# Makiato1999/HRI-EMO

Measured on AMD Instinct MI355X. Metric: utterances/sec fwd+bwd, d=768 T_a=400 T_t=128 N_e=6, higher is better.
Workload: dtype bf16; 1 GPU; FusionWithEmotionDecoder fwd+bwd (train mode, dropout 0.1), d=768 T_a=400 T_t=128 N_e=6 H=8, 2 fusion + 2 decoder layers, all-False masks (BASELINE cfg2); global_batch=64, batch_per_gpu=64, parallelism=dp1, grad_allreduce=none, launch=hipGraph replay, streams=2

## Files before the change

### hri-emo_amd/_lib.py

```python
import ctypes
import os

_HERE = os.path.dirname(os.path.abspath(__file__))
LIB_PATH = os.environ.get("HRIEMO_LIB") or os.path.join(_HERE, "libhriemo.so")

_C = {"p": ctypes.c_void_p, "i": ctypes.c_int, "l": ctypes.c_long, "f": ctypes.c_float,
      "Q": ctypes.c_ulonglong, "I": ctypes.c_uint}

_SIGS = {
    "hriemo_gemm_bf16": ("iiiiiplplplipipliplp", "i"),
    "hriemo_gemm_force_config": ("i", "i"),
    "hriemo_gemm_debug_flags": ("i", "i"),
    "hriemo_gemm_colsum_rows": ("iiiii", "i"),
    "hriemo_gemm_plan": ("iiiiiilppp", "i"),
    "hriemo_gemm_bf16_group_tn": ("piip", "i"),
    "hriemo_gemm_bf16_split": ("iiiiiplplplpliiplp", "i"),
    "hriemo_gemm_bf16_colsum": ("iiiiiplplplplpp", "i"),
    "hriemo_mx8_scale_ld": ("i", "l"),
    "hriemo_quant_mx8": ("pliiiplplp", "i"),
    "hriemo_gemm_mx8": ("iiiplplplplplipiplp", "i"),
    "hriemo_gemm_mx8_q": ("iiiplplplplplpiplplp", "i"),
    "hriemo_gemm_mx8_force_config": ("i", "i"),
    "hriemo_attn_fwd": ("plplplplppiiiiifQpIipp", "i"),
    "hriemo_attn_fwd_q": ("plplplplppiiiiifQpIipplplp", "i"),
    "hriemo_attn_bwd": ("plplplplplplplplpppiiiiifQpIipppp", "i"),
    "hriemo_attn_fwd_varlen": ("plplplplpppiiiiifQpIipp", "i"),
    "hriemo_attn_fwd_q_varlen": ("plplplplpppiiiiifQpIipplpllp", "i"),
    "hriemo_attn_bwd_varlen": ("plplplplplplplplppppiiiiifQpIipppp", "i"),
    "hriemo_attn_mask_bytes": ("iiii", "l"),
    "hriemo_attn_bwd_single_pass": ("iiii", "i"),
    "hriemo_attn_bwd_single_pass_q": ("iiiii", "i"),
    "hriemo_attn_bwd_kv_colsum_rows": ("iiiii", "i"),
    "hriemo_attn_bwd_colsum_rows": ("iiii", "i"),
    "hriemo_attn_bwd_dq_colsum_rows": ("iiiii", "i"),
    "hriemo_attn_plan": ("iiiiiipppppp", "i"),
    "hriemo_split_bf16x3": ("pliipiip", "i"),
    "hriemo_attn_fwd_f32": ("plplplplppiiiiifQpIip", "i"),
    "hriemo_attn_probs_f32": ("plplpppiiiiifQpIip", "i"),
    "hriemo_add_ln_f32": ("ppppppiiffQpIlp", "i"),
    "hriemo_dropout_f32": ("ppliipfQpIlp", "i"),
    "hriemo_masked_mean_f32": ("pppiiip", "i"),
    "hriemo_gate_input_f32": ("pppiip", "i"),
    "hriemo_sigmoid_beta_f32": ("pppiip", "i"),
    "hriemo_fuse_f32": ("ppipippiiip", "i"),
    "hriemo_split3_f32": ("pliipiiplp", "i"),
    "hriemo_colsum_f32_workspace_bytes": ("ii", "l"),
    "hriemo_colsum_f32": ("pliiplpipp", "i"),
    "hriemo_add_ln_bwd_f32_workspace_bytes": ("ii", "l"),
    "hriemo_add_ln_bwd_f32": ("pppppppppiiiffQpIlpp", "i"),
    "hriemo_attn_bwd_f32": ("plplplplplppplplplpiiiiifQpIip", "i"),
    "hriemo_gate_dpre_f32": ("ppipipppiiip", "i"),
    "hriemo_gate_input_bwd_f32": ("pppppiip", "i"),
    "hriemo_gate_dy_f32": ("ppipppiiiip", "i"),
    "hriemo_rowdot_bwd_f32": ("ppppppiiip", "i"),
    "hriemo_attn_fwd_f32_varlen": ("plplplplpppiiiiifQpIip", "i"),
    "hriemo_attn_bwd_f32_varlen": ("plplplplplpppplplplpiiiiifQpIip", "i"),
    "hriemo_add_ln_f32_rows": ("ppppppiiffQpIlpp", "i"),
    "hriemo_add_ln_bwd_f32_rows": ("pppppppppiiiffQpIlppp", "i"),
    "hriemo_masked_mean_f32_packed": ("ppipiiip", "i"),
    "hriemo_fuse_f32_packed": ("pppiippiipppiiiip", "i"),
    "hriemo_gate_dpre_f32_packed": ("ppippiippiipppiiip", "i"),
    "hriemo_gate_dy_f32_packed": ("ppipippipiiiip", "i"),
    "hriemo_attn_probs": ("plplpppiiiiifQpIip", "i"),
    "hriemo_attn_probs_mfma": ("plplpppiiiiifQpIip", "i"),
    "hriemo_attn_probs_varlen": ("plplppppiiiiiiifQpIip", "i"),
    "hriemo_attn_probs_f32_varlen": ("plplppppiiiiiiifQpIip", "i"),
    "hriemo_add_ln_fwd": ("pppppppppiiffQpIlp", "i"),
    "hriemo_add_ln_fwd_mx8": ("pppppppppiiffQpIlpplp", "i"),
    "hriemo_add_ln_fwd_rows": ("pppppppppiiffQpIlpplpp", "i"),
    "hriemo_add_ln_bwd_rows": ("ppppppppppppiiifQpIlppp", "i"),
    "hriemo_add_ln_bwd_workspace_bytes": ("ii", "l"),
    "hriemo_add_ln_bwd": ("ppppppppppppiiifQpIlpp", "i"),
    "hriemo_colsum_workspace_bytes": ("ii", "l"),
    "hriemo_colsum_bf16": ("pliipipp", "i"),
    "hriemo_cast_f32_to_bf16": ("pplp", "i"),
    "hriemo_cast_bf16_to_f32": ("pplp", "i"),
    "hriemo_cast_f32_to_bf16_batch": ("pip", "i"),
    "hriemo_cast_copy_batch": ("pip", "i"),
    "hriemo_pack_rows": ("pppiiiipppp", "i"),
    "hriemo_unpack_rows": ("pppiiippp", "i"),
    "hriemo_dropout_bf16": ("pplifQpIlp", "i"),
    "hriemo_gemm_ln_supported": ("i", "i"),
    "hriemo_gemm_ln_fwd": ("iiiplplppppppppppffQpIlpp", "i"),
    "hriemo_expand_rows": ("pppilp", "i"),
    "hriemo_seed_bump": ("pp", "i"),
    "hriemo_rowdot_fwd": ("pppppiip", "i"),
    "hriemo_rowdot_bwd": ("pppppppiiip", "i"),
    "hriemo_pool_chunks": ("i", "i"),
    "hriemo_ln_pool_fwd": ("pppppppppiiiifp", "i"),
    "hriemo_gate_input": ("ppppiiiipppp" + "p", "i"),
    "hriemo_sigmoid_beta": ("pppiip", "i"),
    "hriemo_fuse_fwd": ("ppppiiip", "i"),
    "hriemo_add_ln_bwd_partial_rows": ("ii", "i"),
    "hriemo_rowops_force_variant": ("i", "i"),
    "hriemo_colsum_partial_rows": ("ii", "i"),
    "hriemo_colreduce_batch": ("pipip", "i"),
    "hriemo_debug_hog": ("iipp", "i"),
    "hriemo_sumsq_f32": ("plpip", "i"),
    "hriemo_adamw_flat": ("pppplfffffifpp", "i"),
    "hriemo_optim_finalize": ("pippppp", "i"),
    "hriemo_adamw_flat_dev": ("pppplppp", "i"),
    "hriemo_masked_mean_fwd": ("ppppiiip", "i"),
    "hriemo_rowsum_f32": ("ppilp", "i"),
    "hriemo_gate_input_pooled": ("pppiip", "i"),
    "hriemo_fusion_loss": ("ppppiiiffpppp", "i"),
    "hriemo_fusion_loss_ce": ("pppiiiffpppp", "i"),
    "hriemo_scalar_gate_dx": ("pipippppiiip", "i"),
    "hriemo_fuse_bwd_dw": ("ppppiiip", "i"),
    "hriemo_gate_dpre": ("pippp" + "iip", "i"),
    "hriemo_gate_input_bwd": ("ppppppiip", "i"),
    "hriemo_ln_pool_bwd_chunks": ("i", "i"),
    "hriemo_ln_pool_pair_supported": ("i", "i"),
    "hriemo_ln_pool_fwd_pair": ("pppppppppi" * 2 + "iiifp", "i"),
    "hriemo_ln_pool_bwd_pair": ("pip" + "ppppppppppip" * 2 + "iiip", "i"),
    "hriemo_ln_pool_bwd_workspace_bytes": ("iii", "l"),
    "hriemo_ln_pool_bwd": ("pipipppppppppp" + "iiiipp", "i"),
    "hriemo_ln_pool_fwd_packed": ("pppiippppppipiiifp", "i"),
    "hriemo_ln_pool_fwd_packed_pair": ("pppiippppppi" * 2 + "piiifp", "i"),
    "hriemo_fuse_fwd_packed": ("pppppiiiip", "i"),
    "hriemo_fuse_fwd_packed_q": ("pppppiiiipplp", "i"),
    "hriemo_fuse_bwd_dw_packed": ("pppppiiiip", "i"),
    "hriemo_ln_pool_bwd_packed": ("ppipippppiipppppp" + "iiiipp", "i"),
    "hriemo_ln_pool_bwd_packed_pair": ("ppip" + "ppppiippppppip" * 2 + "iiip", "i"),
    "hriemo_prof_enable": ("i", "i"),
    "hriemo_prof_nclass": ("", "i"),
    "hriemo_prof_collect": ("ippp", "i"),
    "hriemo_abi_version": ("", "i"),
}

_lib = None


def lib():
    global _lib
    if _lib is None:
        if not os.path.exists(LIB_PATH):
            raise RuntimeError(
                f"{LIB_PATH} not found: build it with `make -C hri-emo_amd/csrc` (or __graft_entry__.build()). "
                "There is no CPU/eager fallback for this path.")
        L = ctypes.CDLL(LIB_PATH)
        for name, (args, res) in _SIGS.items():
            fn = getattr(L, name)
            fn.argtypes = [_C[c] for c in args]
            fn.restype = _C[res]
        L.hriemo_last_error.restype = ctypes.c_char_p
        L.hriemo_last_error.argtypes = []
        L.hriemo_prof_name.restype = ctypes.c_char_p
        L.hriemo_prof_name.argtypes = [ctypes.c_int]
        _lib = L
    return _lib


def call(name, *args):
    L = lib()
    rc = getattr(L, name)(*args)
    if rc != 0:
        raise RuntimeError(f"{name} failed ({rc}): {L.hriemo_last_error().decode()}")
```

### hri-emo_amd/_ops.py

```python
import itertools
import os as _os
import threading
from collections import namedtuple

import torch

from . import _lib

BF16 = torch.bfloat16
_EPS = 1e-5
_apply_tls = threading.local()


def _stream():
    return torch.cuda.current_stream().cuda_stream


def _p(t):
    return None if t is None else t.data_ptr()


def _require_fp32_master(p):
    if p.dtype != torch.float32:
        raise TypeError(f"hri_emo_amd: parameter of dtype {p.dtype}; keep the module's parameters in fp32 "
                        "(the bf16 compute copies are made internally, as under torch.autocast)")


def _require_fp32_masters(*ps):
    for p in ps:
        if p is not None:
            _require_fp32_master(p)


def _require_gpu(t):
    if not t.is_cuda:
        raise RuntimeError(
            "hri_emo_amd runs on MI355X only: got a CPU tensor. There is no CPU fallback for this path "
            "(move the module and its inputs to 'cuda').")


_ws_cache = {}
_ws_retired = []
GRAPHS_ALIVE = 0


def workspace(nbytes, device, slot=0):
    key = (device.index, slot, torch.cuda.current_stream(device).cuda_stream)
    t = _ws_cache.get(key)
    if t is None or t.numel() * 4 < nbytes:
        if t is not None and GRAPHS_ALIVE > 0:
            _ws_retired.append(t)
        n = max(int(nbytes), 64 << 20) // 4 + 16
        t = torch.empty(n, dtype=torch.float32, device=device)
        _ws_cache[key] = t
    return t


_side_streams = {}
TWO_STREAMS = _os_env_flag = None


def side_stream(device):
    global TWO_STREAMS
    if TWO_STREAMS is None:
        import os
        TWO_STREAMS = os.environ.get("HRIEMO_TWO_STREAMS", "1") != "0"
    if not TWO_STREAMS:
        return None
    s = _side_streams.get(device.index)
    if s is None:
        s = torch.cuda.Stream(device=device)
        _side_streams[device.index] = s
    return s


class StepContext:
    __slots__ = ("capturing", "capture_origin", "seq_override", "join_scope", "half_reports")

    def __init__(self):
        self.capturing, self.capture_origin, self.seq_override, self.join_scope, self.half_reports = False, None, None, 0, {}


CTX = StepContext()


class use_context:

    def __init__(self, ctx):
        self.ctx, self.prev = ctx, None

    def __enter__(self):
        global CTX
        self.prev, CTX = CTX, self.ctx
        return self.ctx

    def __exit__(self, *exc):
        global CTX
        CTX = self.prev
        return False


def fork(child, parent):
    if CTX.capturing and CTX.capture_origin is not None and parent != CTX.capture_origin and child != CTX.capture_origin:
        raise RuntimeError("hri_emo_amd: a stream was forked from a stream that is itself a fork of the capture stream; ROCm 7.2 "
                           "crashes in hipStreamEndCapture on nested forks -- fork helper streams from the capturing stream only "
                           "(join the side stream back first), or run this step eagerly")
    child.wait_stream(parent)


_main_streams = {}


def note_main_stream(stream):
    _main_streams[stream.device.index] = stream


def branch_streams(device):
    out = [_main_streams.get(device.index, torch.cuda.current_stream(device))]
    side = _side_streams.get(device.index)
    if side is not None:
        out.append(side)
    return out


def share(t, stream):
    if t is not None:
        t.record_stream(stream)
    return t


class TextBranch:

    def __init__(self, side, main):
        self.side, self.main = side, main

    def fork(self, *handed):
        if self.side is not None:
            fork(self.side, self.main)
            for x in handed:
                share(x, self.side)

    def run(self):
        return torch.cuda.stream(self.side)

    def join(self, *back):
        if self.side is not None:
            self.main.wait_stream(self.side)
            for x in back:
                share(x, self.main)


_site_counter = itertools.count(1)


def new_site_base():
    return next(_site_counter) * 4


_seed_words = {}
STEP_ID = 0


def begin_step():
# ... 216 lines not shown
                    if (p.dim() < 2 or any(p is q for q in after_flush)) and _small_dw.touches(p.grad):
                        _small_dw.add_hook(hook, p, True)
                    elif (p.dim() < 2 or any(p is q for q in after_flush)) and DEFER_REDUCE and _in_backward():
                        _deferred.add_hook(hook, p)
                    elif p.dim() >= 2 and _small_dw.touches(p.grad):
                        _small_dw.add_hook(hook, p)
                    else:
                        hook(p)


def prefetch_batch(pairs):
    jobs, upd = [], []
    for sh, p in pairs:
        need, dst, ver = sh.stale(p)
        if not need:
            continue
        _require_gpu(p)
        _require_fp32_master(p)
        if not p.is_contiguous() or p.data_ptr() % 16:
            sh.get(p)
            continue
        if dst is None:
            dst = torch.empty(p.shape, dtype=BF16, device=p.device)
        jobs.append((p.data_ptr(), dst.data_ptr(), p.numel()))
        upd.append((sh, id(p), ver, dst))
    if jobs:
        host = torch.tensor(jobs, dtype=torch.int64)
        _lib.call("hriemo_cast_f32_to_bf16_batch", host.data_ptr(), len(jobs), _stream())
        for sh, key, ver, dst in upd:
            sh._d[key] = (ver, dst, STEP_ID)


def padded_shadow(sh, p, kp):
    key = (id(p), "pad")
    ent = sh._d.get(key)
    ver = (p._version, p.data_ptr(), WEIGHTS_EPOCH)
    if CTX.capturing or ent is None or ent[0] != ver or ent[1].device != p.device:
        _require_gpu(p)
        _require_fp32_master(p)
        s_ = ent[1] if ent is not None and ent[1].device == p.device else \
            torch.zeros((p.shape[0], kp), dtype=BF16, device=p.device)
        s_[:, :p.shape[1]].copy_(p.detach())
        ent = (ver, s_)
        sh._d[key] = ent
    return ent[1]


def to_bf16(x):
    return x if x.dtype == BF16 else x.to(BF16)


def mask_u8(mask, B, L):
    if mask is None:
        return None
    if mask.shape != (B, L):
        raise ValueError(f"key_padding_mask shape {tuple(mask.shape)} != {(B, L)}")
    m = mask.contiguous()
    return m.view(torch.uint8) if m.dtype == torch.bool else m.to(torch.uint8)


def gemm(ta, tb, M, N, K, A, lda, B, ldb, C, ldc, c_f32=False, bias=None, epi=0, aux=None, ldaux=0, accumulate=False):
    ws = workspace(64 << 20, C.device) if c_f32 else None
    _lib.call("hriemo_gemm_bf16", ta, tb, M, N, K, _p(A), lda, _p(B), ldb, _p(C), ldc, int(c_f32), _p(bias), epi,
              _p(aux), ldaux, int(accumulate), _p(ws), ws.numel() * 4 if ws is not None else 0, _stream())


def linear_fwd(x, w16, bias, relu=False, out_f32=False):
    M, K = x.shape
    N = w16.shape[0]
    y = torch.empty((M, N), dtype=torch.float32 if out_f32 else BF16, device=x.device)
    gemm(0, 0, M, N, K, x, x.stride(0), w16, w16.stride(0), y, N, c_f32=out_f32, bias=bias, epi=1 if relu else 0)
    return y


def linear_dx(dy, w16, epi=0, aux=None):
    M, N = dy.shape
    K = w16.shape[1]
    dx = torch.empty((M, K), dtype=BF16, device=dy.device)
    gemm(0, 1, M, K, N, dy, dy.stride(0), w16, w16.stride(0), dx, K, epi=epi, aux=aux,
         ldaux=aux.stride(0) if aux is not None else 0)
    return dx


FOLD_FFN_BIAS = True


def fold_ffn_bias():
    return FOLD_FFN_BIAS


def linear_dx_masked_colsum(dy, w16, aux, bias_out, accumulate):
    M, N = dy.shape
    K = w16.shape[1]
    dx = torch.empty((M, K), dtype=BF16, device=dy.device)
    rows = _lib.lib().hriemo_gemm_colsum_rows(0, 1, M, K, N)
    part = torch.empty(rows * K, dtype=torch.float32, device=dy.device)
    _lib.call("hriemo_gemm_bf16_colsum", 0, 1, M, K, N, _p(dy), dy.stride(0), _p(w16), w16.stride(0), _p(dx), K, _p(aux), aux.stride(0),
              _p(part), _stream())
    if accumulate and DEFER_REDUCE and _in_backward():
        _deferred.add(part, K, rows, K, 1, [bias_out], True)
    else:
        red = _DeferredReduce()
        red.device = dy.device
        red.add(part, K, rows, K, 1, [bias_out], accumulate, schedule=False)
        red.flush()
    return dx


def linear_dw(dy, x, out, accumulate=False):
    M, N = dy.shape
    K = x.shape[1]
    if accumulate and M <= SMALL_DW_ROWS and _small_dw.enabled():
        _small_dw.add(dy, x, out)
        return
    gemm(1, 1, N, K, M, dy, dy.stride(0), x, x.stride(0), out, out.stride(0), c_f32=True, accumulate=accumulate)


def linear_dw_split(dy, x, out, out2, split, accumulate=False):
    M, N = dy.shape
    K = x.shape[1]
    ws = workspace(64 << 20, out.device)
    _lib.call("hriemo_gemm_bf16_split", 1, 1, N, K, M, _p(dy), dy.stride(0), _p(x), x.stride(0), _p(out), out.stride(0), _p(out2),
              out2.stride(0), split, int(accumulate), _p(ws), ws.numel() * 4, _stream())


GEMM_MODE = None


def set_gemm_mode(mode):
    global GEMM_MODE
    if mode not in ("bf16", "mx_fp8"):
        raise ValueError(f"gemm mode {mode!r}: expected 'bf16' or 'mx_fp8'")
    GEMM_MODE = mode


def gemm_mode():
    global GEMM_MODE
    if GEMM_MODE is None:
        import os
        GEMM_MODE = os.environ.get("HRIEMO_GEMM", "bf16")
        if GEMM_MODE not in ("bf16", "mx_fp8"):
            raise ValueError(f"HRIEMO_GEMM={GEMM_MODE!r}: expected 'bf16' or 'mx_fp8'")
    return GEMM_MODE


PRECISION = None


def set_precision(mode):
    global PRECISION
    if mode not in ("bf16", "fp32"):
        raise ValueError(f"set_precision: {mode!r} (expected 'bf16' or 'fp32')")
    PRECISION = mode


def precision():
    global PRECISION
    if PRECISION is None:
        import os
        mode = os.environ.get("HRIEMO_PRECISION", "bf16")
        if mode not in ("bf16", "fp32"):
            raise ValueError(f"HRIEMO_PRECISION={mode!r} (expected 'bf16' or 'fp32')")
        PRECISION = mode
    return PRECISION


# ... 248 lines not shown
    if cu is not None:
        out = torch.empty((B,) + tuple(out_l), dtype=torch.float32, device=q.device)
        _lib.call("hriemo_attn_probs_varlen", _p(q), q.stride(0), _p(k), k.stride(0), _p(cu[0]), _p(cu[1]), _p(lse), _p(out), B, H,
                  Lq, Lk, out_l[0], out_l[1], hd, float(p), seed, _p(seed_word(q.device)), site, b_off, _stream())
        return out
    out = torch.empty((B, Lq, Lk), dtype=torch.float32, device=q.device)
    _lib.call("hriemo_attn_probs_mfma" if MFMA_MAPS else "hriemo_attn_probs", _p(q), q.stride(0), _p(k), k.stride(0), _p(kpm), _p(lse), _p(out), B, H, Lq, Lk,
              hd, float(p), seed, _p(seed_word(q.device)), site, b_off, _stream())
    return out


def add_ln_fwd(g, x, gamma, beta, p, seed, site, row_off, x32=None, want32=False, want_mx=False, rows=None):
    M, d = g.shape
    y = torch.empty((M, d), dtype=BF16, device=g.device)
    y32 = torch.empty((M, d), dtype=torch.float32, device=g.device) if want32 else None
    mean = torch.empty(M, dtype=torch.float32, device=g.device)
    rstd = torch.empty(M, dtype=torch.float32, device=g.device)
    if DROP_LOG is not None and p > 0 and rows is None:
        DROP_LOG.append(("rows", seed, site, M, d, float(p), row_off))
    if rows is not None:
        yq = ys = None
        ld = 0
        if want_mx:
            ld = _lib.lib().hriemo_mx8_scale_ld(M)
            yq = torch.empty((M, d), dtype=torch.uint8, device=g.device)
            ys = torch.empty((d // 32, ld), dtype=torch.uint8, device=g.device)
        _lib.call("hriemo_add_ln_fwd_rows", _p(g), _p(x), _p(x32), _p(gamma), _p(beta), _p(y), _p(y32), _p(mean), _p(rstd), M, d,
                  _EPS, float(p), seed, _p(seed_word(g.device)), site, row_off, _p(yq), _p(ys), ld, _p(rows), _stream())
        return (y, y32, mean, rstd, (yq, ys)) if want_mx else (y, y32, mean, rstd)
    if want_mx:
        ld = _lib.lib().hriemo_mx8_scale_ld(M)
        yq = torch.empty((M, d), dtype=torch.uint8, device=g.device)
        ys = torch.empty((d // 32, ld), dtype=torch.uint8, device=g.device)
        _lib.call("hriemo_add_ln_fwd_mx8", _p(g), _p(x), _p(x32), _p(gamma), _p(beta), _p(y), _p(y32), _p(mean), _p(rstd), M, d,
                  _EPS, float(p), seed, _p(seed_word(g.device)), site, row_off, _p(yq), _p(ys), ld, _stream())
        return y, y32, mean, rstd, (yq, ys)
    _lib.call("hriemo_add_ln_fwd", _p(g), _p(x), _p(x32), _p(gamma), _p(beta), _p(y), _p(y32), _p(mean), _p(rstd), M, d,
              _EPS, float(p), seed, _p(seed_word(g.device)), site, row_off, _stream())
    return y, y32, mean, rstd


def add_ln_bwd(dy, g, x, gamma, mean, rstd, p, seed, site, row_off, want_dx=True, outs=None, accumulate=False, x32=None, rows=None):
    M, d = g.shape
    dev = g.device
    dx = torch.empty((M, d), dtype=BF16, device=dev) if want_dx else None
    dg = torch.empty((M, d), dtype=BF16, device=dev) if (p > 0 or not want_dx) else None
    if outs is None:
        stats = torch.empty((3, d), dtype=torch.float32, device=dev)
        outs = (stats[0], stats[1], stats[2])
    L_ = _lib.lib()
    defer = accumulate and DEFER_REDUCE and _in_backward()
    if defer:
        nparts = L_.hriemo_add_ln_bwd_partial_rows(M, d)
        ws = torch.empty(nparts * 3 * d, dtype=torch.float32, device=dev)
        dests = (None, None, None, 0)
    else:
        ws = workspace(L_.hriemo_add_ln_bwd_workspace_bytes(M, d), dev, slot=1)
        dests = (_p(outs[0]), _p(outs[1]), _p(outs[2]), int(accumulate))
    _lib.call("hriemo_add_ln_bwd_rows", _p(dy), _p(g), _p(x), _p(x32), _p(gamma), _p(mean), _p(rstd), _p(dx), _p(dg), *dests, M, d,
              float(p), seed, _p(seed_word(dev)), site, row_off, _p(ws), _p(rows), _stream())
    if defer:
        _deferred.add(ws, 3 * d, nparts, d, 3 if outs[2] is not None else 2, [o for o in outs if o is not None], True)
    if dg is None:
        dg = dx
    return dx, dg, outs[0], outs[1], outs[2]


def ln_pool_fwd(x, x32, sx, gamma, beta, Yn, mean, rstd, part, sf, d):
    if sf.packed:
        _lib.call("hriemo_ln_pool_fwd_packed", _p(x), _p(x32), _p(sx.cu), sx.B, sx.N, _p(gamma), _p(beta), _p(Yn), _p(mean), _p(rstd),
                  _p(part), sx.L, _p(sf.cu), sf.N, sx.Breal, d, _EPS, _stream())
    else:
        _lib.call("hriemo_ln_pool_fwd", _p(x), _p(x32), _p(sx.kpm), _p(gamma), _p(beta), _p(Yn), _p(mean), _p(rstd), _p(part),
                  sx.B, sx.L, sf.L, d, _EPS, _stream())


def ln_pool_fwd_pair(a, t, sf, d):
    if sf.packed:
        side = lambda x, x32, sx, *rest: (_p(x), _p(x32), _p(sx.cu), sx.B, sx.N, *map(_p, rest), sx.L)
        _lib.call("hriemo_ln_pool_fwd_packed_pair", *side(*a), *side(*t), _p(sf.cu), sf.N, a[2].Breal, d, _EPS, _stream())
    else:
        side = lambda x, x32, sx, *rest: (_p(x), _p(x32), _p(sx.kpm), *map(_p, rest), sx.L)
        _lib.call("hriemo_ln_pool_fwd_pair", *side(*a), *side(*t), a[2].B, sf.L, d, _EPS, _stream())


def fuse_fwd(w, An, Tn, H, sf, d):
    if sf.packed and want_mx_copy(sf.N, d):
        ld = _lib.lib().hriemo_mx8_scale_ld(sf.N)
        hq = torch.empty((sf.N, d), dtype=torch.uint8, device=H.device)
        hs = torch.empty((d // 32, ld), dtype=torch.uint8, device=H.device)
        _lib.call("hriemo_fuse_fwd_packed_q", _p(w), _p(An), _p(Tn), _p(H), _p(sf.cu), sf.N, sf.Breal, sf.L, d, _p(hq), _p(hs), ld,
                  _stream())
        tag_mx(H, (hq, hs))
    elif sf.packed:
        _lib.call("hriemo_fuse_fwd_packed", _p(w), _p(An), _p(Tn), _p(H), _p(sf.cu), sf.N, sf.Breal, sf.L, d, _stream())
    else:
        _lib.call("hriemo_fuse_fwd", _p(w), _p(An), _p(Tn), _p(H), sf.B, sf.L, d, _stream())


def fuse_bwd_dw(dH, An, Tn, part, sf, d):
    if sf.packed:
        _lib.call("hriemo_fuse_bwd_dw_packed", _p(dH), _p(An), _p(Tn), _p(part), _p(sf.cu), sf.N, sf.Breal, sf.L, d, _stream())
    else:
        _lib.call("hriemo_fuse_bwd_dw", _p(dH), _p(An), _p(Tn), _p(part), sf.B, sf.L, d, _stream())


def ln_pool_bwd(dH, sf, w, is_a, dpool, x, x32, sx, gamma, mean, rstd, dx, dgamma, dbeta, accumulate, ws, d):
    if sf.packed:
        _lib.call("hriemo_ln_pool_bwd_packed", _p(dH), _p(sf.cu), sf.N, _p(w), is_a, _p(dpool), _p(x), _p(x32), _p(sx.cu), sx.B, sx.N,
                  _p(gamma), _p(mean), _p(rstd), _p(dx), _p(dgamma), _p(dbeta), accumulate, sx.Breal, sx.L, d, _p(ws), _stream())
    else:
        _lib.call("hriemo_ln_pool_bwd", _p(dH), sf.L, _p(w), is_a, _p(dpool), _p(sx.kpm), _p(x), _p(x32), _p(gamma), _p(mean),
                  _p(rstd), _p(dx), _p(dgamma), _p(dbeta), accumulate, sx.B, sx.L, d, _p(ws), _stream())


def ln_pool_bwd_pair(dH, sf, w, a, t, accumulate, d):
    if sf.packed:
        side = lambda ws, dpool, x, x32, sx, *rest: (_p(dpool), _p(x), _p(x32), _p(sx.cu), sx.B, sx.N, *map(_p, rest), sx.L, _p(ws))
        _lib.call("hriemo_ln_pool_bwd_packed_pair", _p(dH), _p(sf.cu), sf.N, _p(w), *side(*a), *side(*t), accumulate, a[4].Breal, d, _stream())
    else:
        side = lambda ws, dpool, x, x32, sx, *rest: (_p(dpool), _p(sx.kpm), _p(x), _p(x32), *map(_p, rest), sx.L, _p(ws))
        _lib.call("hriemo_ln_pool_bwd_pair", _p(dH), sf.L, _p(w), *side(*a), *side(*t), accumulate, a[4].B, d, _stream())


TWIN = _os.environ.get("HRIEMO_FP32_TWIN", "1") != "0"


DEFER_REDUCE = True
FOLD_ATTN_BIAS = True


class _DeferredReduce:

    def __init__(self):
        self.jobs, self.keep, self.scheduled, self.blocks, self.hooks = [], [], False, 0, []

    def _schedule(self):
        if not self.scheduled:
            torch.autograd.Variable._execution_engine.queue_callback(self.flush)
            self.scheduled = True

    def add_hook(self, hook, p):
        self.hooks.append((hook, p))
        self._schedule()

    def add(self, part, pstride, np_, w, nseg, outs, accumulate, schedule=True):
        gx = (w + 31) // 32
        self.jobs.append([part.data_ptr(), pstride, np_, w, nseg | (int(bool(accumulate)) << 8) | (self.blocks << 32)]
                         + [o.data_ptr() for o in outs] + [0] * (3 - len(outs)))
        self.blocks += gx * nseg
        self.keep.append(part)
        self.keep.extend(outs)
        self.device = part.device
        if schedule:
            self._schedule()

    def flush(self):
        jobs, n, nblocks = self.jobs, len(self.jobs), self.blocks
        self.jobs, self.scheduled, self.blocks = [], False, 0
        if n:
            host = torch.tensor(jobs, dtype=torch.int64)
            dev = torch.empty((n, 8), dtype=torch.int64, device=self.device)
            _lib.call("hriemo_colreduce_batch", host.data_ptr(), n, _p(dev), nblocks, _stream())
            self.keep.append(dev)
        if not CTX.capturing and self.keep:
            cur = torch.cuda.current_stream(self.device)
# ... 719 lines not shown
            if dkv is not None:
                dcat[:, d:].copy_(dkv)
        wq, wkv = ctx.params
        sq, skv = GradSink((wq,)), GradSink((wkv,))
        dwq = dwkv = None
        if dq is not None:
            dwq = sq.buf(wq)
            if not sq.fused:
                dwq[d:].zero_()
        if dkv is not None:
            dwkv = skv.buf(wkv)
            if not skv.fused:
                dwkv[:d].zero_()
        if dwq is not None and dwkv is not None and sq.fused == skv.fused:
            linear_dw_split(dcat, x2, dwq[:d], dwkv[d:], d, sq.fused)
        else:
            if dwq is not None:
                linear_dw(dcat[:, :d], x2, dwq[:d], sq.fused)
            if dwkv is not None:
                linear_dw(dcat[:, d:], x2, dwkv[d:], skv.fused)
        dep = None
        if ctx.join is not None:
            _, dep = ctx.join.arrive()
        dx = linear_dx(dcat, wcat, epi=3, aux=dep.view(M, d)) if dep is not None else linear_dx(dcat, wcat)
        _report_half(wq, sq)
        _report_half(wkv, skv)
        return dx.view(B, L, d), (sq.ret(dwq) if dwq is not None else None), None, (skv.ret(dwkv) if dwkv is not None else None), None, None, None, None


class KVProjFn(torch.autograd.Function):

    @staticmethod
    def forward(ctx, xkv, w_in, b_in, sh, join=None):
        _require_fp32_masters(w_in, b_in)
        _require_gpu(xkv)
        ctx.join = join
        B, Lk, d = xkv.shape
        xkv2 = _contig_bf16(xkv).view(B * Lk, d)
        w_in16 = sh.get(w_in)
        kv = proj_fwd(Operand(xkv2, mx_of(xkv)), sh, w_in, w_in16, b_in, rows=(d, 3 * d))
        ctx.save_for_backward(xkv2, w_in16)
        ctx.cfg = (B, Lk, d)
        ctx.params = (w_in,)
        return kv

    @staticmethod
    def backward(ctx, dkv):
        xkv2, w_in16 = ctx.saved_tensors
        B, Lk, d = ctx.cfg
        dkv = _contig_bf16(dkv)
        sink = GradSink(ctx.params)
        acc = sink.fused
        dw_in = sink.buf(ctx.params[0])
        if not acc:
            dw_in[:d].zero_()
        linear_dw(dkv, xkv2, dw_in[d:], acc)
        last, dep = ctx.join.arrive() if ctx.join is not None else (True, None)
        dxkv = linear_dx(dkv, w_in16[d:], epi=3, aux=dep.view(B * Lk, d)) if dep is not None else linear_dx(dkv, w_in16[d:])
        sink.done()
        if not last:
            ctx.join.deposit(dxkv)
            return None, sink.ret(dw_in), None, None, None
        return dxkv.view(B, Lk, d), sink.ret(dw_in), None, None, None


class FFNLN(_GradModeAware, torch.autograd.Function):

    @staticmethod
    def forward(ctx, x, x32, w1, b1, w2, b2, gamma, beta, sh, p, p_mid, seed, site, b_off, seq):
        seq.holds(x)
        if seq.packed and p_mid > 0:
            raise ValueError("FFNLN: packed rows with a mid-FFN dropout are not built (the encoder's FFNs have none)")
        if precision() == "fp32":
            return _fp32().ffn_ln(ctx, x, x32, w1, b1, w2, b2, gamma, beta, sh, p, p_mid, seed, site, b_off, seq)
        _require_fp32_masters(w1, b1, w2, b2, gamma, beta)
        ctx.set_materialize_grads(False)
        _require_gpu(x)
        B, L, d = x.shape
        M = B * L
        x2 = _contig_bf16(x).view(M, d)
        x32 = _c32(x32)
        x32v = x32.view(M, d) if x32 is not None else None
        w1_16, w2_16 = sh.get(w1), sh.get(w2)
        h = proj_fwd(Operand(x2, mx_of(x)), sh, w1, w1_16, b1, relu=True, want_q=p_mid == 0)
        hd_ = h
        if p_mid > 0:
            hd_ = torch.empty_like(h)
            if DROP_LOG is not None:
                DROP_LOG.append(("rows", seed, site + 2, M, h.shape[1], float(p_mid), b_off * L))
            _lib.call("hriemo_dropout_bf16", _p(h), _p(hd_), M, h.shape[1], float(p_mid), seed, _p(seed_word(h.device)),
                      site + 2, b_off * L, _stream())
        g, y, y32, mean, rstd, mx = _proj_ln(hd_, sh, w2, w2_16, b2, x2, x32v, gamma, beta, p, seed, site + 1, b_off * seq.L, seq.idx)
        ctx.save_for_backward(x2, x32v, h, hd_, g, mean, rstd, w1_16, w2_16, gamma)
        ctx.cfg = (B, L, d, p, p_mid, seed, site, b_off)
        ctx.seq = seq
        ctx.params = (w1, b1, w2, b2, gamma, beta)
        return tag_mx(y.view(B, L, d), mx), (y32.view(B, L, d) if y32 is not None else None)

    @staticmethod
    def backward(ctx, dy, dy32):
        if getattr(ctx, "fp32", False):
            return _fp32().ffn_ln_bwd(ctx, dy, dy32)
        x2, x32v, h, hd_, g, mean, rstd, w1_16, w2_16, gamma = ctx.saved_tensors
        B, L, d, p, p_mid, seed, site, b_off = ctx.cfg
        M, F = h.shape
        dev = x2.device
        p_w1, p_b1, p_w2 = ctx.params[:3]
        sink, ds, dg, dgamma, dbeta, db2 = _ln_bwd(ctx.params, dy, dy32, g, x2, x32v, gamma, mean, rstd, p, seed, site + 1,
                                                   b_off * ctx.seq.L, ctx.seq.idx)
        acc = sink.fused
        dw2 = sink.buf(p_w2)
        linear_dw(dg, hd_, dw2, acc)
        db1 = sink.buf(p_b1)
        fold = p_mid == 0 and fold_ffn_bias()
        if fold:
            da = linear_dx_masked_colsum(dg, w2_16, h, db1, acc)
        else:
            da = linear_dx(dg, w2_16, epi=2, aux=h)
        if p_mid > 0:
            _lib.call("hriemo_dropout_bf16", _p(da), _p(da), M, F, float(p_mid), seed, _p(seed_word(dev)), site + 2, b_off * L,
                      _stream())
        dw1 = sink.buf(p_w1)
        linear_dw(da, x2, dw1, acc)
        if not fold:
            colsum(da, db1, acc)
        dx = linear_dx(da, w1_16, epi=3, aux=ds)
        sink.done()
        r = sink.ret
        return (dx.view(B, L, d), None, r(dw1), r(db1), r(dw2), r(db2), r(dgamma), r(dbeta)) + (None,) * 7


class BetaGateFn(_GradModeAware, torch.autograd.Function):

    @staticmethod
    def forward(ctx, h_a, h_a32, h_t, h_t32, ga, ba, gt, bt, w1, b1, w2, b2, sh, sa, st, sf):
        if not (sa.packed == st.packed == sf.packed):
            raise ValueError("BetaGate: the three layouts must be all padded or all packed")
        B, La, Lt, d = sa.Breal, sa.L, st.L, h_a.shape[-1]
        Ra, Rt = h_a.shape[0] * h_a.shape[1], h_t.shape[0] * h_t.shape[1]
        if Ra != sa.N or Rt != st.N:
            raise ValueError(f"BetaGate: packed rows {Ra} / {Rt} do not match the plan ({sa.N} / {st.N})")
        L = La if La == Lt else Lt
        if La < L:
            raise RuntimeError(f"BetaGate: audio length {La} < text length {Lt}; the reference cannot fuse this either")
        if precision() == "fp32":
            return _fp32().beta_gate(ctx, h_a, h_a32, h_t, h_t32, ga, ba, gt, bt, w1, b1, w2, b2, sh, sa, st, sf)
        _require_fp32_masters(ga, ba, gt, bt, w1, b1, w2, b2)
        _require_gpu(h_a)
        h_a32, h_t32 = _c32(h_a32), _c32(h_t32)
        dev = h_a.device
        xa, xt = _contig_bf16(h_a), _contig_bf16(h_t)
        f32 = dict(dtype=torch.float32, device=dev)
        L_ = _lib.lib()
        nca, nct = L_.hriemo_pool_chunks(La), L_.hriemo_pool_chunks(Lt)
        An = torch.empty(sf.shape(d), dtype=BF16, device=dev)
        Tn = torch.empty(sf.shape(d), dtype=BF16, device=dev)
        mean_a, rstd_a = torch.empty(Ra, **f32), torch.empty(Ra, **f32)
        mean_t, rstd_t = torch.empty(Rt, **f32), torch.empty(Rt, **f32)
        pa, pt = torch.empty((B, nca, d), **f32), torch.empty((B, nct, d), **f32)
        st_ = _stream()
        side_a = (xa, h_a32, sa, ga, ba, An, mean_a, rstd_a, pa)
        side_t = (xt, h_t32, st, gt, bt, Tn, mean_t, rstd_t, pt)
        main = torch.cuda.current_stream(dev)
        side = side_stream(dev) if GATE_TWO_STREAMS else None
        if GATE_PAIR and L_.hriemo_ln_pool_pair_supported(d):
            ln_pool_fwd_pair(side_a, side_t, sf, d)
        elif side is not None and side != main:
            fork(side, main)
            with torch.cuda.stream(side):
                ln_pool_fwd(*side_t, sf, d)
            ln_pool_fwd(*side_a, sf, d)
            main.wait_stream(side)
            if not CTX.capturing:
                for t_ in (xt, h_t32, st.kpm, Tn, mean_t, rstd_t, pt):
                    share(t_, side)
        else:
            ln_pool_fwd(*side_a, sf, d)
            ln_pool_fwd(*side_t, sf, d)
        gin = torch.empty((B, 4 * d), dtype=BF16, device=dev)
        a_pool, t_pool = torch.empty((B, d), **f32), torch.empty((B, d), **f32)
        cnt = torch.empty((B, 2), **f32)
        _lib.call("hriemo_gate_input", _p(pa), _p(pt), _p(sa.kpm), _p(st.kpm), B, La, Lt, d, _p(gin), _p(a_pool),
                  _p(t_pool), _p(cnt), st_)
        w1_16, w2_16 = sh.get(w1), sh.get(w2)
        hid = linear_fwd(gin, w1_16, b1, relu=True)
        pre = linear_fwd(hid, w2_16, b2, out_f32=True)
        w = torch.empty((B, d), **f32)
        beta = torch.empty((B, 1), **f32)
        _lib.call("hriemo_sigmoid_beta", _p(pre), _p(w), _p(beta), B, d, st_)
        H = torch.empty(sf.shape(d), dtype=BF16, device=dev)
        fuse_fwd(w, An, Tn, H, sf, d)
        ctx.save_for_backward(xa, xt, An, Tn, mean_a, rstd_a, mean_t, rstd_t, gin, a_pool, t_pool, cnt, hid, w, w1_16,
                              w2_16, ga, gt, h_a32, h_t32)
        ctx.seqs = (sa, st, sf)
        ctx.params = (ga, ba, gt, bt, w1, b1, w2, b2)
        return H, beta

    @staticmethod
    def backward(ctx, dH, dbeta):
        if getattr(ctx, "fp32", False):
            return _fp32().beta_gate_bwd(ctx, dH, dbeta)
        (xa, xt, An, Tn, mean_a, rstd_a, mean_t, rstd_t, gin, a_pool, t_pool, cnt, hid, w, w1_16, w2_16, ga, gt,
         h_a32, h_t32) = ctx.saved_tensors
        sa, st, sf = ctx.seqs
        B, La, Lt, L, d = sa.Breal, sa.L, st.L, st.L, xa.shape[-1]
        dev = xa.device
        f32 = dict(dtype=torch.float32, device=dev)
        st_ = _stream()
        L_ = _lib.lib()
        p_ga, p_ba, p_gt, p_bt, p_w1, p_b1, p_w2, p_b2 = ctx.params
        sink = GradSink(ctx.params)
        acc = sink.fused
        dH2 = _contig_bf16(dH) if dH is not None else torch.zeros(An.shape, dtype=BF16, device=dev)
        dbeta2 = dbeta.contiguous().float() if dbeta is not None else None
        part = torch.empty((B, L_.hriemo_pool_chunks(L), d), **f32)
        fuse_bwd_dw(dH2, An, Tn, part, sf, d)
        dpre = torch.empty((B, d), dtype=BF16, device=dev)
        _lib.call("hriemo_gate_dpre", _p(part), L, _p(dbeta2), _p(w), _p(dpre), B, d, st_)
        dw2 = sink.buf(p_w2)
        linear_dw(dpre, hid, dw2, acc)
        db2 = sink.buf(p_b2)
        colsum(dpre, db2, acc)
        dhid = linear_dx(dpre, w2_16, epi=2, aux=hid)
        dw1 = sink.buf(p_w1)
        linear_dw(dhid, gin, dw1, acc)
        db1 = sink.buf(p_b1)
        colsum(dhid, db1, acc)
        dgin = linear_dx(dhid, w1_16)
        da, dt = torch.empty((B, d), **f32), torch.empty((B, d), **f32)
        _lib.call("hriemo_gate_input_bwd", _p(dgin), _p(a_pool), _p(t_pool), _p(cnt), _p(da), _p(dt), B, d, st_)
        dxa = torch.empty(sa.shape(d), dtype=BF16, device=dev)
        dxt = torch.empty(st.shape(d), dtype=BF16, device=dev)
        dga, dba, dgt, dbt = sink.buf(p_ga), sink.buf(p_ba), sink.buf(p_gt), sink.buf(p_bt)
        defer = acc and DEFER_REDUCE and _in_backward()
        nba, nbt = L_.hriemo_ln_pool_bwd_workspace_bytes(B, La, d), L_.hriemo_ln_pool_bwd_workspace_bytes(B, Lt, d)

        def one_side(is_a, dpool, x, x32, sx, gamma, mean, rstd, dx, dgam, dbet, nbytes):
            wsx = torch.empty(nbytes // 4 + 16, **f32) if defer else workspace(nbytes, dev, slot=1)
            outs_ = (None, None, 1) if defer else (dgam, dbet, int(acc))
            ln_pool_bwd(dH2, sf, w, is_a, dpool, x, x32, sx, gamma, mean, rstd, dx, *outs_, wsx, d)
            if defer:
                _deferred.add(wsx, 2 * d, B * L_.hriemo_ln_pool_bwd_chunks(sx.L), d, 2, [dgam, dbet], True)

        side_a = (da, xa, h_a32, sa, ga, mean_a, rstd_a, dxa)
        side_t = (dt, xt, h_t32, st, gt, mean_t, rstd_t, dxt)
        main = torch.cuda.current_stream(dev)
        side = side_stream(dev) if GATE_TWO_STREAMS else None
        if GATE_PAIR and L_.hriemo_ln_pool_pair_supported(d):
# ... 271 lines not shown
```

### hri-emo_amd/csrc/gemm.hip

```cpp
#include "gemm_common.h"
#include <string.h>
#include <stdlib.h>

template <int TA, int TB, int OUTF32, int BM, int BN, int WM, int WN, int NS, int BK>
__device__ __forceinline__ void gemm_body(const GemmArgs& p) {
  constexpr int NWAVE = WM * WN;
  constexpr bool K32 = (BK == 32), STAG = K32 && (WM * WN == 8);
  constexpr int A_BYTES = BM * BK * 2, B_BYTES = BN * BK * 2, STAGE = A_BYTES + B_BYTES;
  constexpr int A_PW = A_BYTES / 1024 / NWAVE, B_PW = B_BYTES / 1024 / NWAVE, LPT = A_PW + B_PW;
  constexpr int MT = BM / WM / 16, NTL = BN / WN / 16;
  static_assert(A_PW * NWAVE * 1024 == A_BYTES && B_PW * NWAVE * 1024 == B_BYTES, "tile must split evenly over waves");
  static_assert(NS >= 2 && NS <= 8 && (NS - 1) * LPT < 64, "ring depth / vmcnt range");
  static_assert(!STAG || NS == 4, "staggered schedule: 4 ring slots");
  static_assert(!K32 || NS >= 3, "32-deep stages need a ring of 3");
  extern __shared__ __attribute__((aligned(16))) char smem[];
  const int tid = threadIdx.x, lane = tid & 63;
  const int wave = __builtin_amdgcn_readfirstlane(tid >> 6);
  const int wm = wave / WN, wn = wave % WN;
  char* scratch = smem + NS * STAGE + wave * 2048;

  const int G = gridDim.x, nxcd = min(8, G), q = G / nxcd, r = G - q * nxcd;
  const int xcd = blockIdx.x % nxcd, lb = blockIdx.x / nxcd, nx = q + (xcd < r ? 1 : 0);
  const int before = xcd * q + min(xcd, r);
  const int tiles = p.tiles_m * p.tiles_n;
  const long total = (long)tiles * p.splitk;
  const int end = (int)(total * (before + nx) / G);
  const int beg = (int)(total * before / G);
  const bool dyn = p.sched != nullptr;
  unsigned* const qctr = p.sched + xcd;
  int* const qslot = (int*)(smem + NS * STAGE);
  auto leave = [&]() {
    if (dyn && tid == 0) {
      const unsigned done = atomicAdd(p.sched + 8, 1u);
      if (done == gridDim.x - 1) {
#pragma unroll
        for (int k = 0; k < 9; ++k) __hip_atomic_store(p.sched + k, 0u, __ATOMIC_RELAXED, __HIP_MEMORY_SCOPE_AGENT);
      }
    }
  };
  int wg, nwg;
  if (dyn) {
    if (tid == 0) {
      const int first = (int)atomicAdd(qctr, 2u);
      qslot[0] = beg + first;
      qslot[1] = beg + first + 1;
    }
    __syncthreads();
    wg = __builtin_amdgcn_readfirstlane(qslot[0]);
    nwg = __builtin_amdgcn_readfirstlane(qslot[1]);
    __syncthreads();
  } else {
    wg = beg + lb;
    nwg = wg + nx;
  }
  if (wg >= end) { leave(); return; }

  const long astep = TA == 0 ? BK : BK * p.lda, bstep = TB == 0 ? BK : BK * p.ldb;
  const LaneOff aoff = operand_lane<TA, BM, BK>(p.lda, lane), boff = operand_lane<TB, BN, BK>(p.ldb, lane);

  auto decode = [&](int w) {
    TileInfo t;
    t.slice = w / tiles;
    const int r = w - t.slice * tiles;
    const int tm = r / p.tiles_n, tn = r - tm * p.tiles_n;
    t.m0 = tm * BM; t.n0 = tn * BN;
    const int kbeg = t.slice * p.k_per_split;
    t.kext = min(p.K, kbeg + p.k_per_split) - kbeg;
    t.nk = (t.kext + BK - 1) / BK;
    t.abase = TA == 0 ? p.A + (long)t.m0 * p.lda + kbeg : p.A + (long)kbeg * p.lda + t.m0;
    t.bbase = TB == 0 ? p.B + (long)t.n0 * p.ldb + kbeg : p.B + (long)kbeg * p.ldb + t.n0;
    t.a_valid = p.M - t.m0; t.b_valid = p.N - t.n0;
    return t;
  };
  constexpr bool REBUILD = (MT * NTL > 16);
  auto stage = [&](int s, const TileInfo& t, int kstep) {
    char* sa = smem + s * STAGE;
    const int krem = t.kext - kstep * BK;
    if (REBUILD) {
      int l2 = lane;
      asm volatile("" : "+v"(l2));
      const LaneOff ao = operand_lane<TA, BM, BK>(p.lda, l2), bo = operand_lane<TB, BN, BK>(p.ldb, l2);
      stage_operand<TA, BM, A_PW, BK>(sa, t.abase + kstep * astep, ao, p.lda, t.a_valid, krem, wave, lane);
      stage_operand<TB, BN, B_PW, BK>(sa + A_BYTES, t.bbase + kstep * bstep, bo, p.ldb, t.b_valid, krem, wave, lane);
    } else {
      stage_operand<TA, BM, A_PW, BK>(sa, t.abase + kstep * astep, aoff, p.lda, t.a_valid, krem, wave, lane);
      stage_operand<TB, BN, B_PW, BK>(sa + A_BYTES, t.bbase + kstep * bstep, boff, p.ldb, t.b_valid, krem, wave, lane);
    }
  };
// ... 154 lines not shown
            __builtin_amdgcn_s_barrier();
            load_frags(smem + cur * STAGE, 0, afA, bfA);
          } else {
            __builtin_amdgcn_s_waitcnt(0xC07F);
          }
          __builtin_amdgcn_sched_barrier(0);
          __builtin_amdgcn_s_setprio(1);
          mma(afB, bfB);
          __builtin_amdgcn_s_setprio(0);
          __builtin_amdgcn_sched_barrier(0);
        };
        for (int it = 0; it < n_steady; ++it) kstep(it, Steady());
        for (int it = n_steady; it < nk; ++it) kstep(it, Tail());
      } else {
        constexpr int MH = MT / 2;
        bf16x8 a0[MH], a1[MH], b0[NTL], b1[NTL];
        auto load_a = [&](const char* sa, int ks, int half, bf16x8 (&af)[MH]) {
#pragma unroll
          for (int mi = 0; mi < MH; ++mi)
            af[mi] = TA == 0 ? lds_row_frag<BK>(sa, wm * MT * 16 + (half * MH + mi) * 16, ks, lane)
                             : lds_tr_frag<BM * 2>(sa, wm * MT * 16 + (half * MH + mi) * 16, ks, lane);
        };
        auto load_b = [&](const char* sa, int ks, bf16x8 (&bfr)[NTL]) {
          const char* sb = sa + A_BYTES;
#pragma unroll
          for (int ni = 0; ni < NTL; ++ni)
            bfr[ni] = TB == 0 ? lds_row_frag<BK>(sb, wn * NTL * 16 + ni * 16, ks, lane) : lds_tr_frag<BN * 2>(sb, wn * NTL * 16 + ni * 16, ks, lane);
        };
        auto cluster = [&](int half, const bf16x8 (&af)[MH], const bf16x8 (&bfr)[NTL]) {
          __builtin_amdgcn_s_setprio(1);
#pragma unroll
          for (int mi = 0; mi < MH; ++mi)
#pragma unroll
            for (int ni = 0; ni < NTL; ++ni)
              acc[half * MH + mi][ni] = __builtin_amdgcn_mfma_f32_16x16x32_bf16(bfr[ni], af[mi], acc[half * MH + mi][ni], 0, 0, 0);
          __builtin_amdgcn_s_setprio(0);
          __builtin_amdgcn_sched_barrier(0);
        };
        load_a(smem + cur * STAGE, 0, 0, a0);
        load_b(smem + cur * STAGE, 0, b0);
        auto kstep = [&](int it, auto steady) {
          prefetch_s(it, steady);
          const char* sa = smem + cur * STAGE;
          __builtin_amdgcn_sched_barrier(0);
          load_a(sa, 0, 1, a1);
          cluster(0, a0, b0);
          load_a(sa, 1, 0, a0);
          load_b(sa, 1, b1);
          cluster(1, a1, b0);
          load_a(sa, 1, 1, a1);
          cluster(0, a0, b1);
          cur = (cur + 1 == NS) ? 0 : cur + 1;
          nxt = (nxt + 1 == NS) ? 0 : nxt + 1;
          if (decltype(steady)::value || it + 1 < nk) {
            retire_s(it, steady);
            __builtin_amdgcn_s_waitcnt(0xC07F);
            __builtin_amdgcn_s_barrier();
            __builtin_amdgcn_sched_barrier(0);
            load_a(smem + cur * STAGE, 0, 0, a0);
            load_b(smem + cur * STAGE, 0, b0);
          }
          cluster(1, a1, b1);
        };
        for (int it = 0; it < n_steady; ++it) kstep(it, Steady());
        for (int it = n_steady; it < nk; ++it) kstep(it, Tail());
      }
    }
    if (has_next) wait_vmcnt<(NS - 2) * LPT>();
    int drawn = end;
    if (dyn && has_next && tid == 0) drawn = beg + (int)atomicAdd(qctr, 1u);
#if defined(HRIEMO_GEMM_ABL) && (HRIEMO_GEMM_ABL & 8)
    bool skip_epilogue;
    {
      float sum = 0.f;
#pragma unroll
      for (int a = 0; a < MT; ++a)
#pragma unroll
        for (int b = 0; b < NTL; ++b) sum += acc[a][b][0] + acc[a][b][1] + acc[a][b][2] + acc[a][b][3];
      skip_epilogue = sum != 12345.678f;
    }
    if (skip_epilogue) {
    } else
#endif
    if (OUTF32) {
      store_tile<1, 0, MT, NTL>(acc, p, T, scratch, wm, wn, lane);
    } else {
      switch (p.epi) {
        case 1: store_tile<0, 1, MT, NTL>(acc, p, T, scratch, wm, wn, lane); break;
        case 2: store_tile<0, 2, MT, NTL>(acc, p, T, scratch, wm, wn, lane); break;
        case 3: store_tile<0, 3, MT, NTL>(acc, p, T, scratch, wm, wn, lane); break;
        default: store_tile<0, 0, MT, NTL>(acc, p, T, scratch, wm, wn, lane); break;
      }
    }
    if (!has_next) break;
    if (!OUTF32) {
      const int rows_valid = p.M - (T.m0 + wm * MT * 16), cols_valid = p.N - (T.n0 + wn * 64);
      relax_first = (p.flags & 1) && rows_valid >= MT * 16 && cols_valid >= 64 && p.cs == nullptr;
    }
    T = decode(nwg);
    wg = nwg;
    if (dyn) {
      if (tid == 0) qslot[0] = drawn;
      __builtin_amdgcn_s_waitcnt(0xC07F);
      parked = true;
    } else {
      nwg = wg + nx;
    }
  }
  leave();
}

template <int TA, int TB, int OUTF32, int BM, int BN, int WM, int WN, int NS, int BK>
__global__ __launch_bounds__(WM * WN * 64, (WM * WN == 4 ? 2 : 1)) void gemm_kernel(const GemmArgs p) {
  gemm_body<TA, TB, OUTF32, BM, BN, WM, WN, NS, BK>(p);
}

template <int TA, int TB, int OUTF32>
__global__ __launch_bounds__(768) void gemm_ws_kernel(const GemmArgs p) {
  constexpr int BM = 256, BN = 128, BK = 64, NS = 3, WN = 2, NCW = 8, NLW = 4, MT = 4, NTL = 4;
  constexpr int A_BYTES = BM * BK * 2, B_BYTES = BN * BK * 2, STAGE = A_BYTES + B_BYTES;
  constexpr int A_PL = A_BYTES / 1024 / NLW, B_PL = B_BYTES / 1024 / NLW, LPL = A_PL + B_PL;
  extern __shared__ __attribute__((aligned(16))) char smem[];
  const int tid = threadIdx.x, lane = tid & 63;
  const int wave = __builtin_amdgcn_readfirstlane(tid >> 6);
  const int G = gridDim.x, nxcd = min(8, G), q = G / nxcd, r = G - q * nxcd;
  const int xcd = blockIdx.x % nxcd, lb = blockIdx.x / nxcd, nx = q + (xcd < r ? 1 : 0);
  const int before = xcd * q + min(xcd, r);
  const int tiles = p.tiles_m * p.tiles_n;
  const long total = (long)tiles * p.splitk;
  const int end = (int)(total * (before + nx) / G), beg = (int)(total * before / G);
  const bool dyn = p.sched != nullptr;
  unsigned* const qctr = p.sched + xcd;
  int* const qslot = (int*)(smem + NS * STAGE);
  const int wg0 = beg + lb, wg1 = wg0 + nx;
  auto leave = [&]() {
    if (dyn && tid == 0) {
      const unsigned done = atomicAdd(p.sched + 8, 1u);
      if (done == gridDim.x - 1) {
#pragma unroll
        for (int k = 0; k < 9; ++k) __hip_atomic_store(p.sched + k, 0u, __ATOMIC_RELAXED, __HIP_MEMORY_SCOPE_AGENT);
      }
    }
  };
  if (wg0 >= end) { leave(); return; }
  auto decode = [&](int w) {
    TileInfo t;
    t.slice = w / tiles;
    const int rr = w - t.slice * tiles;
    const int tm = rr / p.tiles_n, tn = rr - tm * p.tiles_n;
    t.m0 = tm * BM; t.n0 = tn * BN;
    const int kbeg = t.slice * p.k_per_split;
    t.kext = min(p.K, kbeg + p.k_per_split) - kbeg;
    t.nk = (t.kext + BK - 1) / BK;
    t.abase = TA == 0 ? p.A + (long)t.m0 * p.lda + kbeg : p.A + (long)kbeg * p.lda + t.m0;
    t.bbase = TB == 0 ? p.B + (long)t.n0 * p.ldb + kbeg : p.B + (long)kbeg * p.ldb + t.n0;
    t.a_valid = p.M - t.m0; t.b_valid = p.N - t.n0;
    return t;
  };
  if (wave >= NCW) {
    __builtin_amdgcn_s_setprio(3);
    const int lw = wave - NCW;
    const long astep = TA == 0 ? BK : BK * p.lda, bstep = TB == 0 ? BK : BK * p.ldb;
    const LaneOff aoff = operand_lane<TA, BM, BK>(p.lda, lane), boff = operand_lane<TB, BN, BK>(p.ldb, lane);
    int ik = 0, islot = 0;
    int known_next = dyn ? end : wg1;
    bool more = true, crossed = false;
    TileInfo IT = decode(wg0);
    auto issue_next = [&]() -> bool {
      if (crossed) {
        crossed = false;
        if (known_next < end) IT = decode(known_next); else more = false;
      }
      if (!more) return false;
      char* sa = smem + islot * STAGE;
      const int krem = IT.kext - ik * BK;
      stage_operand<TA, BM, A_PL, BK>(sa, IT.abase + ik * astep, aoff, p.lda, IT.a_valid, krem, lw, lane);
      stage_operand<TB, BN, B_PL, BK>(sa + A_BYTES, IT.bbase + ik * bstep, boff, p.ldb, IT.b_valid, krem, lw, lane);
      islot = (islot + 1 == NS) ? 0 : islot + 1;
      if (++ik == IT.nk) { ik = 0; crossed = true; }
      return true;
    };
    int pending = 0;
    if (issue_next()) ++pending;
    if (issue_next()) ++pending;
    for (int w = wg0; w < end;) {
      const int nk = decode(w).nk;
      for (int it = 0; it < nk; ++it) {
        if (pending >= 2) wait_vmcnt<LPL>(); else wait_vmcnt<0>();
        __builtin_amdgcn_s_barrier();
        if (dyn && it == nk - 2) {
          const int v = *(LDS_PTR(const int))qslot;
          __builtin_amdgcn_s_waitcnt(0xC07F);
          known_next = __builtin_amdgcn_readfirstlane(v);
        }
        --pending;
        if (issue_next()) ++pending;
      }
// ... 270 lines not shown
    const long fit = workspace_bytes > 0 ? workspace_bytes / ((long)M * N * 4) : 0;
    if (want > fit) want = fit;
    if (want > 1) splitk = (int)want;
  }
  const int kper = ((K + splitk - 1) / splitk + 63) / 64 * 64;
  splitk = (K + kper - 1) / kper;
  if (K - (splitk - 1) * kper <= (kCfg[cfg].ns - 2) * kCfg[cfg].bk) cfg = 0;
  return {cfg, splitk, kper};
}
extern "C" int hriemo_gemm_plan(int ta, int tb, int M, int N, int K, int c_is_f32, long workspace_bytes, int* cfg, int* splitk,
                                int* k_per_split) {
  HRIEMO_CHECK(M > 0 && N > 0 && K > 0 && cfg != nullptr && splitk != nullptr && k_per_split != nullptr, "gemm_plan: bad arguments");
  HRIEMO_CHECK(!(ta == 1 && tb == 0), "gemm: layout (ta=1,tb=0) is not used by this path and not built");
  const GemmPlan pl = plan_gemm(ta, tb, M, N, K, c_is_f32, workspace_bytes);
  *cfg = pl.cfg; *splitk = pl.splitk; *k_per_split = pl.k_per_split;
  return 0;
}
extern "C" int hriemo_gemm_colsum_rows(int ta, int tb, int M, int N, int K) {
  const int wr = wave_rows(plan_gemm(ta, tb, M, N, K, 0, 0).cfg);
  return (M + wr - 1) / wr;
}

static int gemm_impl(int ta, int tb, int M, int N, int K, const void* A, long lda, const void* B, long ldb,
                     void* C, long ldc, int c_is_f32, const float* bias, int epilogue, const void* aux,
                     long ldaux, int accumulate, float* workspace, long workspace_bytes, float* colsum_partials, hipStream_t st,
                     void* C2 = nullptr, long ldc2 = 0, int split_m = 0) {
  HRIEMO_CHECK(M > 0 && N > 0 && K > 0, "gemm: empty problem M=%d N=%d K=%d", M, N, K);
  HRIEMO_CHECK(C2 == nullptr || (c_is_f32 && split_m > 0 && split_m < M && ldc2 % 4 == 0 && ((uintptr_t)C2 % 16) == 0),
               "gemm: a split output needs fp32 results, 0 < split_m < M and a 16-byte aligned second matrix");
  HRIEMO_CHECK(!(ta == 1 && tb == 0), "gemm: layout (ta=1,tb=0) is not used by this path and not built");
  HRIEMO_CHECK(N % 8 == 0, "gemm: N=%d must be a multiple of 8", N);
  HRIEMO_CHECK(lda % 8 == 0 && ldb % 8 == 0 && ldc % (c_is_f32 ? 4 : 8) == 0, "gemm: leading dims must keep 16-byte alignment");
  HRIEMO_CHECK(((uintptr_t)A % 16) == 0 && ((uintptr_t)B % 16) == 0 && ((uintptr_t)C % 16) == 0, "gemm: unaligned operand");
  HRIEMO_CHECK(lda < (1L << 21) && ldb < (1L << 21), "gemm: leading dimension too large for 32-bit tile offsets");
  if (ta == 0) HRIEMO_CHECK(K % 8 == 0, "gemm: K=%d must be a multiple of 8 for a K-contiguous operand", K);
  if (ta == 1) HRIEMO_CHECK(M % 8 == 0, "gemm: M=%d must be a multiple of 8 for a transposed A", M);
  HRIEMO_CHECK(c_is_f32 || (epilogue >= 0 && epilogue <= 3), "gemm: bad epilogue");
  HRIEMO_CHECK(epilogue < 2 || (aux != nullptr && ldaux % 8 == 0 && ((uintptr_t)aux % 16) == 0), "gemm: epilogue 2/3 needs a 16-byte aligned aux");
  HRIEMO_CHECK(!(c_is_f32 && epilogue != 0), "gemm: fp32 output has no activation epilogue");
  HRIEMO_CHECK(c_is_f32 || !accumulate, "gemm: accumulate needs fp32 output");

  const GemmPlan pl = plan_gemm(ta, tb, M, N, K, c_is_f32, workspace != nullptr ? workspace_bytes : 0);
  const int cfg = pl.cfg, splitk = pl.splitk;
  GemmArgs a = {};
  a.M = M; a.N = N; a.K = K;
  a.A = (const bf16_t*)A; a.lda = lda; a.B = (const bf16_t*)B; a.ldb = ldb;
  a.C = C; a.ldc = ldc; a.bias = bias; a.aux = (const bf16_t*)aux; a.ldaux = ldaux; a.epi = epilogue;
  a.tiles_m = (M + kCfg[cfg].bm - 1) / kCfg[cfg].bm; a.tiles_n = (N + kCfg[cfg].bn - 1) / kCfg[cfg].bn;
  a.ws = workspace; a.accumulate = accumulate; a.sched = nullptr;
  a.flags = g_gemm_flags;
  a.cs = colsum_partials;
  HRIEMO_CHECK(colsum_partials == nullptr || (epilogue == 2 && !c_is_f32), "gemm: column sums are built for the masked epilogue (2) with bf16 output");
  a.splitk = splitk; a.k_per_split = pl.k_per_split;
  if (C2 != nullptr && splitk == 1) {
    const char* A2 = (const char*)A + (size_t)split_m * 2;
    HRIEMO_CHECK(ta == 1, "gemm: a split output without split-K is built for the weight-gradient layout only");
    int rc = gemm_impl(ta, tb, split_m, N, K, A, lda, B, ldb, C, ldc, 1, nullptr, 0, nullptr, 0, accumulate, workspace, workspace_bytes, nullptr, st);
    if (rc != 0) return rc;
    return gemm_impl(ta, tb, M - split_m, N, K, A2, lda, B, ldb, C2, ldc2, 1, nullptr, 0, nullptr, 0, accumulate, workspace, workspace_bytes, nullptr, st);
  }

  const int cls = ta ? HP_GEMM_TN : (tb ? HP_GEMM_NN : HP_GEMM_NT);
  hriemo_prof_begin(cls, st);
  if (ta == 0 && tb == 0) {
    if (c_is_f32) launch_gemm<0, 0, 1>(a, cfg, st); else launch_gemm<0, 0, 0>(a, cfg, st);
  } else if (ta == 0 && tb == 1) {
    if (c_is_f32) launch_gemm<0, 1, 1>(a, cfg, st); else launch_gemm<0, 1, 0>(a, cfg, st);
  } else {
    if (c_is_f32) launch_gemm<1, 1, 1>(a, cfg, st); else launch_gemm<1, 1, 0>(a, cfg, st);
  }
  HRIEMO_LAUNCH_CHECK("gemm_kernel");
  if (splitk > 1) {
    const long nv = (long)M * N / 4;
    int grid = (int)((nv + 255) / 256);
    if (grid > 16 * hriemo_num_cus()) grid = 16 * hriemo_num_cus();
    hipLaunchKernelGGL(splitk_reduce_kernel, dim3(grid), dim3(256), 0, st, workspace, (float*)C, ldc, M, N, splitk,
                       accumulate, (float*)C2, ldc2, C2 != nullptr ? split_m : M);
    HRIEMO_LAUNCH_CHECK("splitk_reduce_kernel");
  }
  hriemo_prof_end(cls, st, 2.0 * M * N * K);
  return 0;
}

extern "C" int hriemo_gemm_bf16(int ta, int tb, int M, int N, int K, const void* A, long lda, const void* B, long ldb,
                                void* C, long ldc, int c_is_f32, const float* bias, int epilogue, const void* aux,
                                long ldaux, int accumulate, float* workspace, long workspace_bytes, hipStream_t st) {
  return gemm_impl(ta, tb, M, N, K, A, lda, B, ldb, C, ldc, c_is_f32, bias, epilogue, aux, ldaux, accumulate, workspace, workspace_bytes,
                   nullptr, st);
}
extern "C" int hriemo_gemm_bf16_split(int ta, int tb, int M, int N, int K, const void* A, long lda, const void* B, long ldb,
                                      void* C, long ldc, void* C2, long ldc2, int split_m, int accumulate, float* workspace,
                                      long workspace_bytes, hipStream_t st) {
  HRIEMO_CHECK(C2 != nullptr, "gemm_split: second output missing");
  return gemm_impl(ta, tb, M, N, K, A, lda, B, ldb, C, ldc, 1, nullptr, 0, nullptr, 0, accumulate, workspace, workspace_bytes, nullptr, st,
                   C2, ldc2, split_m);
}
extern "C" int hriemo_gemm_bf16_group_tn(const void* jobs_host, int njobs, int accumulate, hipStream_t st) {
  HRIEMO_CHECK(jobs_host != nullptr && njobs > 0, "gemm_group: empty job table");
  const long long* h = (const long long*)jobs_host;
  constexpr int BM = 128, BN = 128;
  using KernelT = void (*)(const GemmGroup);
  KernelT kern = gemm_group_kernel<1, 1, 1, BM, BN, 2, 2, 2, 64>;
  const int lds = kCfg[0].lds + 4 * 2048;
  static bool attr_set = false;
  if (!attr_set) {
    hipFuncSetAttribute((const void*)kern, hipFuncAttributeMaxDynamicSharedMemorySize, lds);
    attr_set = true;
  }
  for (int j0 = 0; j0 < njobs; j0 += 16) {

    GemmGroup g = {};
    const int nj = njobs - j0 < 16 ? njobs - j0 : 16;
    int gx = 1;
    double flops = 0.0;
    for (int j = 0; j < nj; ++j) {
      const long long* r = h + (long)(j0 + j) * 9;
      GemmArgs& a = g.p[j];
      a.M = (int)r[0]; a.N = (int)r[1]; a.K = (int)r[2];
      a.A = (const bf16_t*)r[3]; a.lda = (long)r[4]; a.B = (const bf16_t*)r[5]; a.ldb = (long)r[6]; a.C = (void*)r[7]; a.ldc = (long)r[8];
      HRIEMO_CHECK(a.M > 0 && a.N > 0 && a.K > 0 && a.M % 8 == 0 && a.N % 8 == 0, "gemm_group: job %d: bad shape %dx%dx%d", j0 + j, a.M, a.N, a.K);
      HRIEMO_CHECK(a.lda % 8 == 0 && a.ldb % 8 == 0 && a.ldc % 4 == 0 && ((uintptr_t)a.A % 16) == 0 && ((uintptr_t)a.B % 16) == 0 &&
                       ((uintptr_t)a.C % 16) == 0 && a.lda < (1L << 21) && a.ldb < (1L << 21), "gemm_group: job %d: alignment", j0 + j);
      HRIEMO_CHECK(a.K > (kCfg[0].ns - 2) * kCfg[0].bk, "gemm_group: job %d: reduction too short for the operand ring", j0 + j);
      a.tiles_m = (a.M + BM - 1) / BM; a.tiles_n = (a.N + BN - 1) / BN;
      a.splitk = 1; a.k_per_split = (a.K + 63) / 64 * 64;
      a.accumulate = accumulate; a.sched = nullptr;
      const int tiles = a.tiles_m * a.tiles_n;
      if (tiles > gx) gx = tiles;
      flops += 2.0 * a.M * a.N * a.K;
    }
    for (int j = nj; j < 16; ++j) { g.p[j] = g.p[0]; g.p[j].tiles_m = 0; g.p[j].tiles_n = 0; }
    const int cap = 2 * hriemo_num_cus();
    if (gx > cap) gx = cap;
    hriemo_prof_begin(HP_GEMM_TN, st);
    hipLaunchKernelGGL(kern, dim3(gx, nj), dim3(256), lds, st, g);
    HRIEMO_LAUNCH_CHECK("gemm_group_kernel");
    hriemo_prof_end(HP_GEMM_TN, st, flops);
  }
  return 0;
}
extern "C" int hriemo_gemm_bf16_colsum(int ta, int tb, int M, int N, int K, const void* A, long lda, const void* B, long ldb,
                                       void* C, long ldc, const void* aux, long ldaux, float* colsum_partials, hipStream_t st) {
  HRIEMO_CHECK(colsum_partials != nullptr, "gemm_colsum: partials buffer missing");
  return gemm_impl(ta, tb, M, N, K, A, lda, B, ldb, C, ldc, 0, nullptr, 2, aux, ldaux, 0, nullptr, 0, colsum_partials, st);
}
```

### hri-emo_amd/csrc/gemm_common.h

```cpp
#pragma once
#include "common.h"
#include <mutex>
#include <type_traits>

struct GemmArgs {
  int M, N, K;
  const bf16_t* A; long lda;
  const bf16_t* B; long ldb;
  void* C; long ldc;
  const float* bias;
  const bf16_t* aux; long ldaux;
  int epi;
  int tiles_m, tiles_n, splitk, k_per_split;
  float* ws;
  int accumulate;
  unsigned* sched;
  int flags;
  float* cs;
  const uint8_t* SA; long ldsa;
  const uint8_t* SB; long ldsb;
  uint8_t* CQ; long ldcq;
  uint8_t* SC; long ldsc;
};

unsigned* hriemo_gemm_sched_slot(hipStream_t st);
int hriemo_num_cus();
int hriemo_gemm_debug_flags_get();

__device__ __forceinline__ int swz4(int row) { return (0x78 >> (((row >> 2) & 3) * 2)) & 3; }

template <int BK>
__device__ __forceinline__ bf16x8 lds_row_frag(const char* tile, int sub0, int ks, int lane) {
  const int row = sub0 + (lane & 15);
  if (BK == 64) {
    const int c = ks * 4 + (lane >> 4);
    return *(LDS_PTR(const bf16x8))(tile + row * 128 + ((c ^ (row & 7)) << 4));
  } else {
    const int c = lane >> 4;
    return *(LDS_PTR(const bf16x8))(tile + row * 64 + ((c ^ swz4(row)) << 4));
  }
}

template <int ROWB>
__device__ __forceinline__ bf16x8 lds_tr_frag(const char* tile, int sub0, int ks, int lane) {
  const int g = lane >> 4, i = lane & 15, qq = i >> 2, pp = i & 3;
  const int kr = ks * 32 + 8 * g + qq;
  const int key = qq | ((g & 1) << 2);
  const int c = ((sub0 >> 3) ^ (key << 1)) | (pp >> 1);
  const char* a0 = tile + kr * ROWB + c * 16 + (pp & 1) * 8;
  s16x4 lo = __builtin_amdgcn_ds_read_tr16_b64_v4i16((LDS_PTR(s16x4))a0);
  s16x4 hi = __builtin_amdgcn_ds_read_tr16_b64_v4i16((LDS_PTR(s16x4))(a0 + 4 * ROWB));
  typedef __attribute__((ext_vector_type(8))) short s16x8;
  s16x8 r = {lo[0], lo[1], lo[2], lo[3], hi[0], hi[1], hi[2], hi[3]};
  return __builtin_bit_cast(bf16x8, r);
}

#define OOB_OFF 0x80000000u

struct LaneOff { unsigned a, b; };

__device__ __forceinline__ void lds_dma16(unsigned lds_addr, __attribute__((ext_vector_type(4))) int rsrc, unsigned voff, int soff) {
  asm volatile("s_mov_b32 m0, %0\n\ts_nop 0\n\tbuffer_load_dwordx4 %1, %2, %3 offen lds"
               :
               : "s"(lds_addr), "v"(voff), "s"(rsrc), "s"(soff)
               : "memory", "m0");
}

template <int T, int ROWS, int BK>
__device__ __forceinline__ LaneOff operand_lane(long ld, int lane) {
  LaneOff lo;
  if (T == 0) {
    if (BK == 64) {
      const int row = lane >> 3;
      lo.a = (unsigned)((row * ld + ((lane & 7) ^ row) * 8) * 2);
    } else {
      const int row = lane >> 2;
      lo.a = (unsigned)((row * ld + ((lane & 3) ^ swz4(row)) * 8) * 2);
    }
    lo.b = 0;
  } else {
    constexpr int CPR = ROWS / 8;
    const int lr = lane / CPR, lc = lane % CPR;
    lo.a = (unsigned)(lr * ld * 2);
    lo.b = (unsigned)((lc ^ (lr << 1)) << 4);
  }
  return lo;
}

template <int T, int ROWS, int PW, int BK>
__device__ __forceinline__ void stage_operand(char* tile, const bf16_t* kbase, const LaneOff lo, long ld, int valid, int krem, int wave, int lane) {
  typedef __attribute__((ext_vector_type(4))) int i32x4;
  const unsigned long kb = (unsigned long)kbase;
  const i32x4 rsrc = {(int)(unsigned)kb, (int)((kb >> 32) & 0xffffu), (int)OOB_OFF, 0x00020000};
  const bool full = valid >= ROWS && krem >= BK;
  constexpr int CPR = ROWS / 8;
  constexpr int RPI = 64 / CPR;
  constexpr int RPJ = BK == 64 ? 8 : 16;
  if (full) {
#pragma unroll
    for (int t = 0; t < PW; ++t) {
      const int j = wave * PW + t;
      if (T == 0) {
        lds_dma16((unsigned)(unsigned long)(LDS_PTR(char))(tile + j * 1024), rsrc, lo.a, (int)(j * RPJ * 2 * ld));
      } else {
        const int kr0 = j * RPI;
        const int ukey = (kr0 & 3) | (((kr0 >> 3) & 1) << 2);
        lds_dma16((unsigned)(unsigned long)(LDS_PTR(char))(tile + j * 1024), rsrc, lo.a + (lo.b ^ (unsigned)(ukey << 5)), (int)(kr0 * 2 * ld));
      }
    }
    return;
  }
#pragma unroll
  for (int t = 0; t < PW; ++t) {
    const int j = wave * PW + t;
    unsigned o;
    int so;
    if (T == 0) {
      o = lo.a;
      so = (int)(j * RPJ * 2 * ld);
      const int row = j * RPJ + (BK == 64 ? (lane >> 3) : (lane >> 2));
      const int c = BK == 64 ? ((lane & 7) ^ (row & 7)) : ((lane & 3) ^ swz4(row));
      if (row >= valid || c * 8 >= krem) o = OOB_OFF;
    } else {
      const int kr0 = j * RPI;
      const int ukey = (kr0 & 3) | (((kr0 >> 3) & 1) << 2);
      const unsigned cb = lo.b ^ (unsigned)(ukey << 5);
      o = lo.a + cb;
      so = (int)(kr0 * 2 * ld);
      if ((int)(cb >> 1) >= valid || kr0 + lane / CPR >= krem) o = OOB_OFF;
    }
    lds_dma16((unsigned)(unsigned long)(LDS_PTR(char))(tile + j * 1024), rsrc, o, so);
  }
}

template <int N> __device__ __forceinline__ void wait_vmcnt() { asm volatile("s_waitcnt vmcnt(%0)" ::"n"(N) : "memory"); }

struct TileInfo {
  const bf16_t* abase;
  const bf16_t* bbase;
  int m0, n0, slice, a_valid, b_valid, kext, nk;
};

typedef __attribute__((ext_vector_type(2))) unsigned u32x2;
typedef __attribute__((ext_vector_type(4))) unsigned u32x4;
typedef __attribute__((ext_vector_type(4))) short s16x4v;
typedef __attribute__((ext_vector_type(8))) short s16x8v;

template <int OUTF32, int EPI, int MT, int NTL>
__device__ __forceinline__ void store_tile(f32x4 (&acc)[MT][NTL], const GemmArgs& p, const TileInfo& T, char* scratch,
                                           int wm, int wn, int lane_in) {
  static_assert(NTL == 4, "wave tiles are 64 columns wide");
  int lane = lane_in;
  asm volatile("" : "+v"(lane));
  const int g = lane >> 4, i = lane & 15;
  if (OUTF32) {
#pragma unroll
    for (int mi = 0; mi < MT; ++mi) {
      const int m = T.m0 + wm * MT * 16 + mi * 16 + i;
      if (m >= p.M) continue;
#pragma unroll
      for (int ni = 0; ni < NTL; ++ni) {
        const int n = T.n0 + wn * NTL * 16 + ni * 16 + 4 * g;
        if (n >= p.N) continue;
        f32x4 v = acc[mi][ni];
        if (p.bias != nullptr && T.slice == 0) v += *(const f32x4*)(p.bias + n);
        float* dst = p.splitk > 1 ? p.ws + ((long)T.slice * p.M + m) * p.N + n : (float*)p.C + (long)m * p.ldc + n;
        if (p.splitk == 1 && p.accumulate) v += *(const f32x4*)dst;
        *(f32x4*)dst = v;
      }
    }
  } else {
    const int mb = T.m0 + wm * MT * 16, nb = T.n0 + wn * 64;
    const int rows_valid = p.M - mb, cols_valid = p.N - nb;
    const bool full = rows_valid >= MT * 16 && cols_valid >= 64;
    const int rr = lane >> 3, cc = lane & 7;
    char* cbase = (char*)((bf16_t*)p.C + (long)mb * p.ldc + nb);
    const unsigned line_c = (unsigned)((rr * p.ldc + cc * 8) * 2);

    f32x4 b4[NTL];
#pragma unroll
    for (int ni = 0; ni < NTL; ++ni) {
      const int n = nb + ni * 16 + 4 * g;
      b4[ni] = (p.bias != nullptr && n < p.N) ? *(const f32x4*)(p.bias + n) : (f32x4){0.f, 0.f, 0.f, 0.f};
    }
    constexpr int CM = MT >= 8 ? 2 : MT;
    constexpr int NCH = MT / CM;
    __amdgpu_buffer_rsrc_t rx = __builtin_amdgcn_make_buffer_rsrc((void*)(EPI >= 2 ? p.aux + (long)mb * p.ldaux + nb : (const bf16_t*)p.C), 0, (int)OOB_OFF, 0x00020000);
    const unsigned frag_x = (unsigned)((i * p.ldaux + 4 * g) * 2);
    const unsigned line_x = (cc * 8 < cols_valid) ? (unsigned)((rr * p.ldaux + cc * 8) * 2) : OOB_OFF;
    u32x2 ax[2][EPI == 3 ? CM : 1][NTL];
    u32x4 al[2][EPI == 2 ? CM : 1][2];
    auto load_chunk = [&](int c, int buf) {
#pragma unroll
      for (int q = 0; q < CM; ++q) {
        const int mi = c * CM + q;
        if (EPI == 3) {
#pragma unroll
          for (int ni = 0; ni < NTL; ++ni) {
            const bool ok = full || (mi * 16 + i < rows_valid && ni * 16 + 4 * g < cols_valid);
            ax[buf][q][ni] = __builtin_amdgcn_raw_buffer_load_b64(rx, ok ? (int)frag_x : (int)OOB_OFF, (int)((mi * 16 * p.ldaux + ni * 16) * 2), 0);
          }
        }
        if (EPI == 2) {
#pragma unroll
          for (int k = 0; k < 2; ++k) {
            const bool ok = full || mi * 16 + k * 8 + rr < rows_valid;
            al[buf][q][k] = __builtin_amdgcn_raw_buffer_load_b128(rx, ok ? (int)line_x : (int)OOB_OFF, (int)((mi * 16 + k * 8) * p.ldaux * 2), 0);
          }
        }
      }
    };
    char* wr = scratch + i * 128 + (g & 1) * 8;
    const int wsw = i & 7, gh = g >> 1;
    const char* rd0 = scratch + rr * 128 + ((cc ^ rr) << 4);
    if (EPI >= 2) load_chunk(0, 0);
    float cs8[EPI == 2 ? 8 : 1];
#pragma unroll
    for (int e = 0; e < (EPI == 2 ? 8 : 1); ++e) cs8[e] = 0.f;
#pragma unroll
    for (int c = 0; c < NCH; ++c) {
      if (EPI >= 2 && c + 1 < NCH) load_chunk(c + 1, (c + 1) & 1);
#pragma unroll
      for (int q = 0; q < CM; ++q) {
        const int mi = c * CM + q;
#pragma unroll
        for (int ni = 0; ni < NTL; ++ni) {
          f32x4 v = acc[mi][ni] + b4[ni];
          if (EPI == 3) {
            const bf16x4 a4 = __builtin_bit_cast(bf16x4, ax[c & 1][q][ni]);
#pragma unroll
            for (int e = 0; e < 4; ++e) v[e] += (float)a4[e];
          }
          bf16x4 o = __builtin_convertvector(v, bf16x4);
          if (EPI == 1) {
            const s16x4v z = {0, 0, 0, 0};
            o = __builtin_bit_cast(bf16x4, __builtin_elementwise_max(__builtin_bit_cast(s16x4v, o), z));
          }
          *(LDS_PTR(bf16x4))(wr + (((ni * 2 + gh) ^ wsw) << 4)) = o;
        }
        asm volatile("s_waitcnt lgkmcnt(0)" ::: "memory");
        u32x4 ln[2];
#pragma unroll
        for (int k = 0; k < 2; ++k) ln[k] = *(LDS_PTR(const u32x4))(rd0 + k * 1024);
#pragma unroll
        for (int k = 0; k < 2; ++k) {
          u32x4 v = ln[k];
          if (EPI == 2) {
            const s16x8v z = {0, 0, 0, 0, 0, 0, 0, 0};
            const s16x8v neg = __builtin_elementwise_sub_sat(z, __builtin_bit_cast(s16x8v, al[c & 1][q][k]));
            v &= __builtin_bit_cast(u32x4, neg >> 15);
            asm volatile("" : "+v"(v));
            if (p.cs != nullptr) {
              const bf16x8 m8 = __builtin_bit_cast(bf16x8, v);
#pragma unroll
              for (int e = 0; e < 8; ++e) cs8[e] += (float)m8[e];
            }
          }
          const bool ok = mi * 16 + k * 8 + rr < rows_valid && cc * 8 < cols_valid;
          if (full || ok) *(u32x4*)(cbase + (long)((mi * 16 + k * 8) * p.ldc * 2) + line_c) = v;
          if (EPI <= 1 && p.CQ != nullptr) {
            float f8[8];
            bf8_to_f32(__builtin_bit_cast(bf16x8, v), f8);
            int e;
            const __attribute__((ext_vector_type(2))) int w8 = mx8_block(f8, e);
            const long qrow = mb + mi * 16 + k * 8 + rr;
            const int qcol = nb + cc * 8;
            if (full || ok) {
              *(__attribute__((ext_vector_type(2))) int*)(p.CQ + qrow * p.ldcq + qcol) = w8;
              if ((cc & 3) == 0) p.SC[(long)(qcol >> 5) * p.ldsc + qrow] = (uint8_t)e;
            }
          }
        }
      }
    }
    if (EPI == 2 && p.cs != nullptr) {
#pragma unroll
      for (int e = 0; e < 8; ++e) {
        float t = cs8[e];
        t += __shfl_xor(t, 8);
        t += __shfl_xor(t, 16);
        t += __shfl_xor(t, 32);
        cs8[e] = t;
      }
      if (rr == 0 && mb < p.M && cc * 8 < cols_valid) {
        float* row = p.cs + (long)(mb / (MT * 16)) * p.N + nb + cc * 8;
        *(f32x4*)row = (f32x4){cs8[0], cs8[1], cs8[2], cs8[3]};
        *(f32x4*)(row + 4) = (f32x4){cs8[4], cs8[5], cs8[6], cs8[7]};
      }
    }
  }
}
```

### hri-emo_amd/csrc/rowops.hip

```cpp
#include "common.h"
#include <string.h>
#include <stdlib.h>

#define EPS_DEFAULT 1e-5f

struct RowDrop { uint64_t seed; const unsigned long long* seed_dev; uint32_t site, thr16; float inv_keep; const long long* rowmap; };
static RowDrop row_drop(float p, uint64_t seed, const unsigned long long* seed_dev, uint32_t site) {
  DropCfg d = make_drop(p, seed, site);
  RowDrop r; r.seed = seed; r.seed_dev = seed_dev; r.site = site; r.thr16 = d.thr16; r.inv_keep = d.inv_keep; r.rowmap = nullptr;
  return r;
}
__device__ __forceinline__ uint32_t row_key(const RowDrop& dr) {
  return dr.thr16 != 0 ? site_key(eff_seed(dr.seed, dr.seed_dev), dr.site, 0u) : 0u;
}

template <int NCH>
__device__ __forceinline__ void block_colsum(float* lds_row, const float (&acc)[NCH][8], int nchunk, int lane, int wave, int nwave) {
  for (int w = 0; w < nwave; ++w) {
    if (wave == w) {
#pragma unroll
      for (int c = 0; c < NCH; ++c) {
        const int ch = lane + 64 * c;
        if (ch < nchunk) {
#pragma unroll
          for (int j = 0; j < 8; ++j) {
            if (w == 0) lds_row[ch * 8 + j] = acc[c][j];
            else lds_row[ch * 8 + j] += acc[c][j];
          }
        }
      }
    }
    __syncthreads();
  }
}

__device__ __forceinline__ void row_keep8(uint32_t key32, uint32_t thr16, uint32_t row, int ch, bool (&kp)[8]) {
  if (thr16 == 0) {
#pragma unroll
    for (int j = 0; j < 8; ++j) kp[j] = true;
    return;
  }
  const uint32_t hb = drop_base(key32, row, (uint32_t)(ch * 4));
#pragma unroll
  for (int pr = 0; pr < 4; ++pr) {
    const uint32_t x = mix24(hb + (uint32_t)pr * DROP_CB);
    kp[2 * pr] = keep_lo(x, thr16);
    kp[2 * pr + 1] = keep_hi(x, thr16);
  }
}

__device__ __forceinline__ void load_resid(const bf16_t* X, const float* X32, long off, float* xf) {
  if (X32 != nullptr) {
    const f32x4 a = *(const f32x4*)(X32 + off), b = *(const f32x4*)(X32 + off + 4);
    xf[0] = a[0]; xf[1] = a[1]; xf[2] = a[2]; xf[3] = a[3]; xf[4] = b[0]; xf[5] = b[1]; xf[6] = b[2]; xf[7] = b[3];
  } else if (X != nullptr) {
    bf8_to_f32(*(const bf16x8*)(X + off), xf);
  } else {
#pragma unroll
    for (int j = 0; j < 8; ++j) xf[j] = 0.f;
  }
}

template <int NCH>
__device__ __forceinline__ void load_cols(const float* __restrict__ v, int nchunk, int lane, float (&out)[NCH][8]) {
#pragma unroll
  for (int c = 0; c < NCH; ++c) {
    const int ch = lane + 64 * c;
#pragma unroll
    for (int j = 0; j < 8; ++j) out[c][j] = 0.f;
    if (ch < nchunk) {
      const f32x4 a = *(const f32x4*)(v + ch * 8), b = *(const f32x4*)(v + ch * 8 + 4);
#pragma unroll
      for (int e = 0; e < 4; ++e) { out[c][e] = a[e]; out[c][4 + e] = b[e]; }
    }
  }
}

template <int NCH>
__global__ __launch_bounds__(256) void add_ln_fwd_kernel(const bf16_t* __restrict__ G, const bf16_t* __restrict__ X,
                                                         const float* __restrict__ X32, const float* __restrict__ gamma,
                                                         const float* __restrict__ beta, bf16_t* __restrict__ Y,
                                                         float* __restrict__ Y32, float* __restrict__ mean_o,
                                                         float* __restrict__ rstd_o, int M, int d, float eps, RowDrop dr,
                                                         long row_offset, uint8_t* __restrict__ Yq, uint8_t* __restrict__ SY, long ldsy) {
  const uint32_t key32 = row_key(dr);
// ... 571 lines not shown
    for (int c = 0; c < NCH; ++c) {
      const int ch = lane + 64 * c;
      if (ch < nchunk) load_resid(X, X32, (xbase + l) * d + ch * 8, dst[c]);
    }
  };
  if (PF && chunk * 32 + wave < lend) load_row(chunk * 32 + wave, nx);
  for (int l = chunk * 32 + wave; l < lend; l += 4) {
    const long row = xbase + l;
    float s[NCH][8];
    float sum = 0.f;
    if (!PF) load_row(l, nx);
#pragma unroll
    for (int c = 0; c < NCH; ++c) {
      const int ch = lane + 64 * c;
      if (ch < nchunk) {
#pragma unroll
        for (int j = 0; j < 8; ++j) { s[c][j] = nx[c][j]; sum += s[c][j]; }
      }
    }
    if (PF && l + 4 < lend) load_row(l + 4, nx);
    const float mu = wave_sum(sum) * invd;
    float sq = 0.f;
#pragma unroll
    for (int c = 0; c < NCH; ++c)
      if (lane + 64 * c < nchunk) {
#pragma unroll
        for (int j = 0; j < 8; ++j) { const float t = s[c][j] - mu; sq += t * t; }
      }
    const float rstd = rsqrtf(wave_sum(sq) * invd + eps);
    const bool valid = PK || mask == nullptr || mask[row] == 0;
#pragma unroll
    for (int c = 0; c < NCH; ++c) {
      const int ch = lane + 64 * c;
      if (ch < nchunk) {
        float o[8];
#pragma unroll
        for (int j = 0; j < 8; ++j) {
          o[j] = (s[c][j] - mu) * rstd * (HOIST ? gm8[HOIST ? c : 0][j] : gamma[ch * 8 + j]) + (HOIST ? bt8[HOIST ? c : 0][j] : beta[ch * 8 + j]);
          if (valid) acc[c][j] += o[j];
        }
        if (l < Lkeep) *(bf16x8*)(Yn + (ybase + l) * d + ch * 8) = f32_to_bf8(o);
      }
    }
    if (lane == 0) { mean_o[row] = mu; rstd_o[row] = rstd; }
  }
  block_colsum<NCH>(red, acc, nchunk, lane, wave, 4);
  float* out = partials + ((long)b * nchunks + chunk) * d;
  for (int t = threadIdx.x; t < d; t += 256) out[t] = red[t];
}
template <int NCH, bool PF>
__global__ __launch_bounds__(256) void ln_pool_fwd_kernel(const bf16_t* __restrict__ X, const float* __restrict__ X32, const uint8_t* __restrict__ mask,
                                                          const float* __restrict__ gamma, const float* __restrict__ beta,
                                                          bf16_t* __restrict__ Yn, float* __restrict__ mean_o, float* __restrict__ rstd_o,
                                                          float* __restrict__ partials, int L, int Lkeep, int d, float eps) {
  ln_pool_fwd_body<NCH, PF>(X, X32, mask, gamma, beta, Yn, mean_o, rstd_o, partials, L, Lkeep, d, eps, blockIdx.x, gridDim.x);
}
struct PoolFwdSide { const bf16_t* X; const float* X32; const uint8_t* mask; const float* gamma; const float* beta; bf16_t* Yn; float* mean; float* rstd; float* partials; int L, Lkeep, nc; };
struct PoolFwdPair { PoolFwdSide s[2]; };
#define PAIR_PICK(f) (second ? p.s[1].f : p.s[0].f)
template <int NCH, bool PF>
__global__ __launch_bounds__(256, 4) void ln_pool_fwd_pair_kernel(const PoolFwdPair p, int d, float eps) {
  const bool second = (int)blockIdx.x >= p.s[0].nc;
  ln_pool_fwd_body<NCH, PF>(PAIR_PICK(X), PAIR_PICK(X32), PAIR_PICK(mask), PAIR_PICK(gamma), PAIR_PICK(beta), PAIR_PICK(Yn), PAIR_PICK(mean),
                            PAIR_PICK(rstd), PAIR_PICK(partials), PAIR_PICK(L), PAIR_PICK(Lkeep), d, eps,
                            (int)blockIdx.x - (second ? p.s[0].nc : 0), PAIR_PICK(nc));
}
template <int NCH, bool PF>
__global__ __launch_bounds__(256) void ln_pool_fwd_packed_kernel(const bf16_t* __restrict__ X, const float* __restrict__ X32,
                                                                 const float* __restrict__ gamma, const float* __restrict__ beta,
                                                                 bf16_t* __restrict__ Yn, float* __restrict__ mean_o, float* __restrict__ rstd_o,
                                                                 float* __restrict__ partials, int L, int d, float eps, const PackedArgs pk) {
  ln_pool_fwd_body<NCH, PF, true>(X, X32, nullptr, gamma, beta, Yn, mean_o, rstd_o, partials, L, 0, d, eps, blockIdx.x, gridDim.x, pk);
}
struct PoolFwdSidePk { const bf16_t* X; const float* X32; const int* cu; const float* gamma; const float* beta; bf16_t* Yn; float* mean; float* rstd; float* partials; int L, nc, nseq, n_rows; };
struct PoolFwdPairPk { PoolFwdSidePk s[2]; };
template <int NCH, bool PF>
__global__ __launch_bounds__(256, 4) void ln_pool_fwd_packed_pair_kernel(const PoolFwdPairPk p, const int* __restrict__ cu_f, int n_f, int B, int d, float eps) {
  const bool second = (int)blockIdx.x >= p.s[0].nc;
  if ((int)blockIdx.y > PAIR_PICK(nseq)) return;
  const PackedArgs pk{PAIR_PICK(cu), PAIR_PICK(nseq), PAIR_PICK(n_rows), cu_f, n_f, B};
  ln_pool_fwd_body<NCH, PF, true>(PAIR_PICK(X), PAIR_PICK(X32), nullptr, PAIR_PICK(gamma), PAIR_PICK(beta), PAIR_PICK(Yn), PAIR_PICK(mean),
                                  PAIR_PICK(rstd), PAIR_PICK(partials), PAIR_PICK(L), 0, d, eps,
                                  (int)blockIdx.x - (second ? p.s[0].nc : 0), PAIR_PICK(nc), pk);
}

__global__ __launch_bounds__(256) void gate_input_kernel(const float* __restrict__ pa, int nca, const float* __restrict__ pt, int nct,
                                                         const uint8_t* __restrict__ mask_a, const uint8_t* __restrict__ mask_t, int La, int Lt,
                                                         int d, bf16_t* __restrict__ gin, float* __restrict__ a_pool, float* __restrict__ t_pool,
                                                         float* __restrict__ cnt) {
  __shared__ float sc[2], wc[4][2];
  const int b = blockIdx.x, tid = threadIdx.x;
  float ca = 0.f, ct = 0.f;
  for (int l = tid; l < La; l += 256) ca += (mask_a == nullptr || mask_a[(long)b * La + l] == 0) ? 1.f : 0.f;
  for (int l = tid; l < Lt; l += 256) ct += (mask_t == nullptr || mask_t[(long)b * Lt + l] == 0) ? 1.f : 0.f;
  ca = wave_sum(ca); ct = wave_sum(ct);
  if ((tid & 63) == 0) { wc[tid >> 6][0] = ca; wc[tid >> 6][1] = ct; }
  __syncthreads();
  if (tid == 0) {
    sc[0] = fmaxf(wc[0][0] + wc[1][0] + wc[2][0] + wc[3][0], 1.f); sc[1] = fmaxf(wc[0][1] + wc[1][1] + wc[2][1] + wc[3][1], 1.f);
    cnt[b * 2] = sc[0]; cnt[b * 2 + 1] = sc[1];
  }
  __syncthreads();
  const float ia = 1.f / sc[0], it = 1.f / sc[1];
  for (int c = tid; c < d; c += 256) {
    float a = 0.f, t = 0.f;
    for (int k0 = 0; k0 < nca; k0 += 8) {
      float v[8];
#pragma unroll
      for (int k = 0; k < 8; ++k) v[k] = k0 + k < nca ? pa[((long)b * nca + k0 + k) * d + c] : 0.f;
#pragma unroll
      for (int k = 0; k < 8; ++k) if (k0 + k < nca) a += v[k];
    }
    for (int k0 = 0; k0 < nct; k0 += 8) {
      float v[8];
#pragma unroll
      for (int k = 0; k < 8; ++k) v[k] = k0 + k < nct ? pt[((long)b * nct + k0 + k) * d + c] : 0.f;
#pragma unroll
      for (int k = 0; k < 8; ++k) if (k0 + k < nct) t += v[k];
    }
    a *= ia; t *= it;
    a_pool[(long)b * d + c] = a; t_pool[(long)b * d + c] = t;
    bf16_t* g = gin + (long)b * 4 * d;
    g[c] = (bf16_t)a; g[d + c] = (bf16_t)t; g[2 * d + c] = (bf16_t)fabsf(a - t); g[3 * d + c] = (bf16_t)(a * t);
  }
}

__global__ __launch_bounds__(256) void sigmoid_beta_kernel(const float* __restrict__ pre, float* __restrict__ w, float* __restrict__ beta, int d) {
  __shared__ float red[4];
  const int b = blockIdx.x, tid = threadIdx.x;
  float s = 0.f;
  for (int c = tid; c < d; c += 256) {
    const float v = 1.f / (1.f + __expf(-pre[(long)b * d + c]));
    w[(long)b * d + c] = v;
    s += v;
  }
  s = wave_sum(s);
  if ((tid & 63) == 0) red[tid >> 6] = s;
  __syncthreads();
  if (tid == 0) beta[b] = (red[0] + red[1] + red[2] + red[3]) / (float)d;
}

__global__ void fuse_fwd_kernel(const float* __restrict__ w, const bf16_t* __restrict__ A, const bf16_t* __restrict__ T,
                                bf16_t* __restrict__ H, int B, int L, int d) {
  const int nch = d >> 3;
  const long nv = (long)B * L * nch;
  for (long v = (long)blockIdx.x * blockDim.x + threadIdx.x; v < nv; v += (long)gridDim.x * blockDim.x) {
    const int ch = (int)(v % nch);
    const long b = v / ((long)L * nch);
    float a[8], t[8], o[8];
    bf8_to_f32(*(const bf16x8*)(A + v * 8), a);
    bf8_to_f32(*(const bf16x8*)(T + v * 8), t);
    const float* wp = w + b * d + ch * 8;
#pragma unroll
    for (int j = 0; j < 8; ++j) o[j] = wp[j] * a[j] + (1.f - wp[j]) * t[j];
    *(bf16x8*)(H + v * 8) = f32_to_bf8(o);
  }
}

template <int NCH, bool MXQ = false>
__global__ __launch_bounds__(256) void fuse_fwd_packed_kernel(const float* __restrict__ w, const bf16_t* __restrict__ A, const bf16_t* __restrict__ T,
                                                              bf16_t* __restrict__ H, const int* __restrict__ cu_f, int n_f, int B, int L, int d,
                                                              uint8_t* __restrict__ Hq = nullptr, uint8_t* __restrict__ Hs = nullptr, long lds = 0) {
  typedef __attribute__((ext_vector_type(2))) int i32x2;
  const int lane = threadIdx.x & 63, wave = threadIdx.x >> 6;
  const int b = blockIdx.y, chunk = blockIdx.x, nchunk = d >> 3;
  if (b == B) {
// ... 753 lines not shown
                                                                bf16_t* __restrict__ gin, int d) {
  const int b = blockIdx.x;
  bf16_t* g = gin + (long)b * 4 * d;
  for (int c = threadIdx.x; c < d; c += 256) {
    const float a = a_pool[(long)b * d + c], t = t_pool[(long)b * d + c];
    g[c] = (bf16_t)a; g[d + c] = (bf16_t)t; g[2 * d + c] = (bf16_t)fabsf(a - t); g[3 * d + c] = (bf16_t)(a * t);
  }
}

__global__ __launch_bounds__(256) void sumsq_f32_kernel(const float* __restrict__ x, long n, float* __restrict__ partial) {
  __shared__ float red[4];
  float s = 0.f;
  const long nv = n >> 2;
  for (long v = (long)blockIdx.x * 256 + threadIdx.x; v < nv; v += (long)gridDim.x * 256) {
    const f32x4 t = *(const f32x4*)(x + v * 4);
    s += t[0] * t[0] + t[1] * t[1] + t[2] * t[2] + t[3] * t[3];
  }
  s = wave_sum(s);
  if ((threadIdx.x & 63) == 0) red[threadIdx.x >> 6] = s;
  __syncthreads();
  if (threadIdx.x == 0) partial[blockIdx.x] = red[0] + red[1] + red[2] + red[3];
}

__global__ __launch_bounds__(256) void adamw_flat_kernel(float* __restrict__ p, const float* __restrict__ g, float* __restrict__ m,
                                                         float* __restrict__ v, long n, float lr, float b1, float b2, float eps,
                                                         float wd, float bc1, float bc2, float max_norm, const float* __restrict__ norm2) {
  float coef = 1.f;
  if (max_norm > 0.f) coef = fminf(1.f, max_norm / (sqrtf(norm2[0]) + 1e-6f));
  const float step = lr / bc1, isb2 = 1.f / sqrtf(bc2);
  const long nv = n >> 2;
  for (long i = (long)blockIdx.x * 256 + threadIdx.x; i < nv; i += (long)gridDim.x * 256) {
    f32x4 pp = *(const f32x4*)(p + i * 4), mm = *(const f32x4*)(m + i * 4), vv = *(const f32x4*)(v + i * 4);
    const f32x4 gg = *(const f32x4*)(g + i * 4) * coef;
#pragma unroll
    for (int e = 0; e < 4; ++e) {
      pp[e] *= 1.f - lr * wd;
      mm[e] += (gg[e] - mm[e]) * (1.f - b1);
      vv[e] = vv[e] * b2 + gg[e] * gg[e] * (1.f - b2);
      pp[e] -= step * mm[e] / (sqrtf(vv[e]) * isb2 + eps);
    }
    *(f32x4*)(p + i * 4) = pp; *(f32x4*)(m + i * 4) = mm; *(f32x4*)(v + i * 4) = vv;
  }
}

extern "C" int hriemo_pool_chunks(int L) { return (L + 31) / 32; }

extern "C" int hriemo_ln_pool_fwd(const void* X, const float* X32, const unsigned char* mask, const float* gamma, const float* beta, void* Yn,
                                  float* mean, float* rstd, float* partials, int B, int L, int Lkeep, int d, float eps,
                                  hipStream_t st) {
  if (check_rows(B * L, d)) return 1;
  HRIEMO_CHECK(Lkeep >= 0 && Lkeep <= L, "ln_pool_fwd: Lkeep=%d out of range (L=%d)", Lkeep, L);
  const int nc = (L + 31) / 32;
  hriemo_prof_begin(HP_ROWOPS, st);
#define CALL(N)                                                                                                                  \
  if ((N) <= 2)                                                                                                                  \
    hipLaunchKernelGGL((ln_pool_fwd_kernel<N, ((N) <= 2)>), dim3(nc, B), dim3(256), d * 4, st, (const bf16_t*)X, X32, mask, gamma, beta, (bf16_t*)Yn, mean, rstd, partials, L, Lkeep, d, eps); \
  else                                                                                                                           \
    hipLaunchKernelGGL((ln_pool_fwd_kernel<N, false>), dim3(nc, B), dim3(256), d * 4, st, (const bf16_t*)X, X32, mask, gamma, beta, (bf16_t*)Yn, mean, rstd, partials, L, Lkeep, d, eps)
  DISPATCH_NCH(d, CALL)
#undef CALL
  HRIEMO_LAUNCH_CHECK("ln_pool_fwd_kernel");
  hriemo_prof_end(HP_ROWOPS, st, ((double)B * L + (double)B * Lkeep) * d * 2);
  return 0;
}

extern "C" int hriemo_ln_pool_pair_supported(int d) { return d % 8 == 0 && d <= 1024 ? 1 : 0; }
extern "C" int hriemo_ln_pool_fwd_pair(const void* Xa, const float* Xa32, const unsigned char* mask_a, const float* gamma_a, const float* beta_a,
                                       void* Yna, float* mean_a, float* rstd_a, float* partials_a, int La,
                                       const void* Xt, const float* Xt32, const unsigned char* mask_t, const float* gamma_t, const float* beta_t,
                                       void* Ynt, float* mean_t, float* rstd_t, float* partials_t, int Lt,
                                       int B, int Lkeep, int d, float eps, hipStream_t st) {
  if (check_rows(B * La, d) || check_rows(B * Lt, d)) return 1;
  HRIEMO_CHECK(Lkeep >= 0 && Lkeep <= La && Lkeep <= Lt, "ln_pool_fwd_pair: Lkeep=%d out of range (La=%d, Lt=%d)", Lkeep, La, Lt);
  HRIEMO_CHECK(hriemo_ln_pool_pair_supported(d), "ln_pool_fwd_pair: d=%d (pairs are built for d <= 1024; use two hriemo_ln_pool_fwd calls)", d);
  PoolFwdPair p;
  p.s[0] = PoolFwdSide{(const bf16_t*)Xa, Xa32, mask_a, gamma_a, beta_a, (bf16_t*)Yna, mean_a, rstd_a, partials_a, La, Lkeep, (La + 31) / 32};
  p.s[1] = PoolFwdSide{(const bf16_t*)Xt, Xt32, mask_t, gamma_t, beta_t, (bf16_t*)Ynt, mean_t, rstd_t, partials_t, Lt, Lkeep, (Lt + 31) / 32};
  const int nc = p.s[0].nc + p.s[1].nc;
  hriemo_prof_begin(HP_ROWOPS, st);
  if (d <= 512) hipLaunchKernelGGL((ln_pool_fwd_pair_kernel<1, true>), dim3(nc, B), dim3(256), d * 4, st, p, d, eps);
  else hipLaunchKernelGGL((ln_pool_fwd_pair_kernel<2, true>), dim3(nc, B), dim3(256), d * 4, st, p, d, eps);
  HRIEMO_LAUNCH_CHECK("ln_pool_fwd_pair_kernel");
  hriemo_prof_end(HP_ROWOPS, st, ((double)B * (La + Lt) + 2.0 * B * Lkeep) * d * 2);
  return 0;
}

extern "C" int hriemo_gate_input(const float* partials_a, const float* partials_t, const unsigned char* mask_a,
                                 const unsigned char* mask_t, int B, int La, int Lt, int d, void* gate_in, float* a_pool,
                                 float* t_pool, float* cnt, hipStream_t st) {
  HRIEMO_CHECK(B > 0 && d > 0, "gate_input: empty");
  hipLaunchKernelGGL(gate_input_kernel, dim3(B), dim3(256), 0, st, partials_a, (La + 31) / 32, partials_t, (Lt + 31) / 32, mask_a,
                     mask_t, La, Lt, d, (bf16_t*)gate_in, a_pool, t_pool, cnt);
  HRIEMO_LAUNCH_CHECK("gate_input_kernel");
  return 0;
}

extern "C" int hriemo_sigmoid_beta(const float* pre, float* w, float* beta, int B, int d, hipStream_t st) {
  HRIEMO_CHECK(B > 0 && d > 0, "sigmoid_beta: empty");
  hipLaunchKernelGGL(sigmoid_beta_kernel, dim3(B), dim3(256), 0, st, pre, w, beta, d);
  HRIEMO_LAUNCH_CHECK("sigmoid_beta_kernel");
  return 0;
}

extern "C" int hriemo_masked_mean_fwd(const void* X, const unsigned char* mask, float* pooled, float* cnt, int B, int L, int d,
                                      hipStream_t st) {
  if (check_rows(B * L, d)) return 1;
  hriemo_prof_begin(HP_ROWOPS, st);
  hipLaunchKernelGGL(masked_mean_fwd_kernel, dim3((d / 8 + 63) / 64, B), dim3(256), 0, st, (const bf16_t*)X, mask, pooled, cnt, L, d);
  HRIEMO_LAUNCH_CHECK("masked_mean_fwd_kernel");
  hriemo_prof_end(HP_ROWOPS, st, 1.0 * B * L * d * 2);
  return 0;
}

extern "C" int hriemo_gate_input_pooled(const float* a_pool, const float* t_pool, void* gate_in, int B, int d, hipStream_t st) {
  HRIEMO_CHECK(B > 0 && d > 0, "gate_input_pooled: empty");
  hipLaunchKernelGGL(gate_input_pooled_kernel, dim3(B), dim3(256), 0, st, a_pool, t_pool, (bf16_t*)gate_in, d);
  HRIEMO_LAUNCH_CHECK("gate_input_pooled_kernel");
  return 0;
}

extern "C" int hriemo_rowsum_f32(const float* x, float* out, int B, long n, hipStream_t st) {
  HRIEMO_CHECK(B > 0 && n > 0, "rowsum_f32: empty problem");
  hipLaunchKernelGGL(rowsum_f32_kernel, dim3(B), dim3(256), 0, st, x, out, n);
  HRIEMO_LAUNCH_CHECK("rowsum_f32_kernel");
  return 0;
}

extern "C" int hriemo_scalar_gate_dx(const void* dH, int Lf, const float* beta, int is_a, const float* dpool, const float* cnt,
                                     const unsigned char* mask, void* dX, int B, int L, int d, hipStream_t st) {
  if (check_rows(B * L, d)) return 1;
  HRIEMO_CHECK(Lf >= 0 && Lf <= L, "scalar_gate_dx: Lf=%d out of range (L=%d)", Lf, L);
  long g = ((long)B * L * (d / 8) + 255) / 256;
  if (g > 8192) g = 8192;
  hriemo_prof_begin(HP_ROWOPS, st);
  hipLaunchKernelGGL(scalar_gate_dx_kernel, dim3((int)g), dim3(256), 0, st, (const bf16_t*)dH, Lf, beta, is_a, dpool, cnt, mask,
                     (bf16_t*)dX, B, L, d);
  HRIEMO_LAUNCH_CHECK("scalar_gate_dx_kernel");
  hriemo_prof_end(HP_ROWOPS, st, 2.0 * B * L * d * 2);
  return 0;
}

extern "C" int hriemo_sumsq_f32(const float* x, long n, float* partial, int nblocks, hipStream_t st) {
  HRIEMO_CHECK(n > 0 && n % 4 == 0 && nblocks > 0 && nblocks <= 4096, "sumsq_f32: n=%ld must be a positive multiple of 4, 0 < nblocks <= 4096", n);
  HRIEMO_CHECK(((uintptr_t)x % 16) == 0, "sumsq_f32: unaligned buffer");
  hipLaunchKernelGGL(sumsq_f32_kernel, dim3(nblocks), dim3(256), 0, st, x, n, partial);
  HRIEMO_LAUNCH_CHECK("sumsq_f32_kernel");
  return 0;
}

extern "C" int hriemo_adamw_flat(float* p, const float* g, float* m, float* v, long n, float lr, float beta1, float beta2, float eps,
                                 float weight_decay, int step, float max_norm, const float* norm2, hipStream_t st) {
  HRIEMO_CHECK(n > 0 && n % 4 == 0 && step >= 1, "adamw_flat: n=%ld must be a positive multiple of 4 and step >= 1", n);
  HRIEMO_CHECK(((uintptr_t)p % 16) == 0 && ((uintptr_t)g % 16) == 0 && ((uintptr_t)m % 16) == 0 && ((uintptr_t)v % 16) == 0, "adamw_flat: unaligned buffer");
  HRIEMO_CHECK(max_norm <= 0.f || norm2 != nullptr, "adamw_flat: clipping needs the squared gradient norm");
  const float bc1 = 1.f - powf(beta1, (float)step), bc2 = 1.f - powf(beta2, (float)step);
  long gsz = (n / 4 + 255) / 256;
  if (gsz > 4096) gsz = 4096;
  hipLaunchKernelGGL(adamw_flat_kernel, dim3((int)gsz), dim3(256), 0, st, p, g, m, v, n, lr, beta1, beta2, eps, weight_decay, bc1, bc2,
                     max_norm, norm2);
  HRIEMO_LAUNCH_CHECK("adamw_flat_kernel");
  return 0;
}

extern "C" int hriemo_fuse_fwd(const float* w, const void* A, const void* T, void* H, int B, int L, int d, hipStream_t st) {
  if (check_rows(B * L, d)) return 1;
  long g = ((long)B * L * (d / 8) + 255) / 256;
// ... 233 lines not shown
```

### hri-emo_amd/models/fusion_with_emotion_decoder.py

```python
import torch
import torch.nn as nn

try:
    from .. import _ops
except ImportError:
    from hri_emo_amd import _ops
from .cross_modal_block_tacfn import CrossModalTransformer
from .beta_gate_tacfn import BetaGate
from .emotion_decoder import EmotionDecoder


class FusionWithEmotionDecoder(nn.Module):
    def __init__(self, d_model: int = 768, num_emotions: int = 4, n_heads: int = 8, num_layers_fusion: int = 2,
                 num_layers_decoder: int = 2, beta_hidden: int = 256, dropout: float = 0.1):
        super().__init__()
        self.cross_modal = CrossModalTransformer(num_layers=num_layers_fusion, d_model=d_model, n_heads=n_heads,
                                                 dropout=dropout)
        self.beta_gate = BetaGate(d_model=d_model, hidden_dim=beta_hidden)
        self.emotion_decoder = EmotionDecoder(d_model=d_model, num_emotions=num_emotions, n_heads=n_heads,
                                              num_layers=num_layers_decoder, dropout=dropout, use_output_layer=True)

    def set_batch_offset(self, offset: int):
        for m in self.modules():
            if hasattr(m, "batch_offset"):
                m.batch_offset = int(offset)

    def _prefetch_shadows(self, device):
        if _ops.precision() != "bf16" or not device.type == "cuda":
            return None
        side = _ops.side_stream(device)
        if side is None:
            return None
        main = torch.cuda.current_stream(device)
        _ops.fork(side, main)
        with torch.cuda.stream(side):
            g = self.beta_gate
            pairs = [(g._sh, g.mlp[0].weight), (g._sh, g.mlp[2].weight)]
            for layer in self.emotion_decoder.layers:
                pairs += [(layer._sh, w) for w in (layer.self_attn.in_proj_weight, layer.self_attn.out_proj.weight,
                                                   layer.cross_attn.in_proj_weight, layer.cross_attn.out_proj.weight,
                                                   layer.linear1.weight, layer.linear2.weight)]
            _ops.prefetch_batch(pairs)
            ev = torch.cuda.Event()
            ev.record(side)
        return ev

    def _ensure_3d(self, x):
        if x.dim() == 2:
            return x.unsqueeze(1)
        if x.dim() == 3:
            return x
        raise ValueError(f"Expected 2D or 3D tensor, got {x.shape}")

    def _build_fused_mask(self, mask_a, mask_t, L_fused):
        if mask_a is None and mask_t is None:
            return None

        def fit(m):
            if m is None:
                return None
            if m.size(1) < L_fused:
                pad = torch.ones(m.size(0), L_fused - m.size(1), dtype=torch.bool, device=m.device)
                return torch.cat([m, pad], dim=1)
            return m[:, :L_fused]

        ma, mt = fit(mask_a), fit(mask_t)
        if ma is None:
            return mt
        if mt is None:
            return ma
        return ma | mt

    def forward(self, h_a, h_t, mask_a=None, mask_t=None, return_attention=False):
        h_a, h_t = self._ensure_3d(h_a), self._ensure_3d(h_t)
        out_dtype = h_a.dtype
        need = bool(return_attention)
        a, a32 = _ops.as_pair(h_a)
        t, t32 = _ops.as_pair(h_t)
        _ops.begin_step()
        may_pack = _ops.varlen() and (not need or _ops.varlen_maps()) and mask_a is not None and mask_t is not None and _ops.packed_tail()
        fused_early = None if may_pack else self._build_fused_mask(mask_a, mask_t, h_t.size(1))
        ready = self._prefetch_shadows(a.device)
        _ops.CTX.join_scope += 1
        try:
            a, a32, t, t32, encoder_attns, seqs = self.cross_modal._fwd_pair(a, a32, t, t32, mask_a, mask_t, need, tail=True)
        finally:
            _ops.CTX.join_scope -= 1
        if ready is not None:
            torch.cuda.current_stream(a.device).wait_event(ready)
        h_fusion, beta = self.beta_gate._fwd_pair(a, a32, t, t32, mask_a, mask_t, seqs)
        sm = seqs[2]
        if not sm.packed:
            sm = sm.with_kpm(fused_early if (fused_early is not None and h_fusion.size(1) == h_t.size(1)) else
                             self._build_fused_mask(mask_a, mask_t, h_fusion.size(1)))
        z, logits, decoder_attns = self.emotion_decoder._fwd(h_fusion, sm, need, out_dtype)
        if return_attention:
            return logits, beta, z, {"encoder": encoder_attns, "decoder": decoder_attns}
        return logits, beta, z
```

### include/hriemo.h

```cpp
#ifndef HRIEMO_H_
#define HRIEMO_H_

#ifdef __cplusplus
extern "C" {
#endif

typedef struct ihipStream_t* hriemo_stream_t;

const char* hriemo_last_error(void);
int hriemo_abi_version(void);

int hriemo_gemm_bf16(int ta, int tb, int M, int N, int K, const void* A, long lda, const void* B, long ldb,
                     void* C, long ldc, int c_is_f32, const float* bias, int epilogue, const void* aux,
                     long ldaux, int accumulate, float* workspace, long workspace_bytes, hriemo_stream_t stream);

int hriemo_gemm_bf16_group_tn(const void* jobs_host, int njobs, int accumulate, hriemo_stream_t stream);
int hriemo_gemm_bf16_split(int ta, int tb, int M, int N, int K, const void* A, long lda, const void* B, long ldb, void* C, long ldc,
                           void* C2, long ldc2, int split_m, int accumulate, float* workspace, long workspace_bytes,
                           hriemo_stream_t stream);
int hriemo_gemm_colsum_rows(int ta, int tb, int M, int N, int K);
int hriemo_gemm_bf16_colsum(int ta, int tb, int M, int N, int K, const void* A, long lda, const void* B, long ldb, void* C, long ldc,
                            const void* aux, long ldaux, float* colsum_partials, hriemo_stream_t stream);
int hriemo_gemm_force_config(int cfg);
int hriemo_gemm_debug_flags(int flags);
int hriemo_gemm_plan(int ta, int tb, int M, int N, int K, int c_is_f32, long workspace_bytes, int* cfg, int* splitk,
                     int* k_per_split);

long hriemo_mx8_scale_ld(int rows);
int hriemo_quant_mx8(const void* X, long ldx, int src_is_f32, int M, int K, void* Xq, long ldq, void* S, long lds,
                     hriemo_stream_t stream);
int hriemo_gemm_mx8(int M, int N, int K, const void* Aq, long lda, const void* SA, long ldsa, const void* Bq, long ldb,
                    const void* SB, long ldsb, void* C, long ldc, int c_is_f32, const float* bias, int epilogue,
                    const void* aux, long ldaux, hriemo_stream_t stream);
int hriemo_gemm_mx8_q(int M, int N, int K, const void* Aq, long lda, const void* SA, long ldsa, const void* Bq, long ldb,
                      const void* SB, long ldsb, void* C, long ldc, const float* bias, int epilogue, void* CQ, long ldcq,
                      void* SC, long ldsc, hriemo_stream_t stream);
int hriemo_gemm_mx8_force_config(int cfg);

int hriemo_attn_fwd(const void* Q, long ldq, const void* K, long ldk, const void* V, long ldv, void* O, long ldo,
                    const unsigned char* key_padding_mask, float* lse, int B, int H, int Lq, int Lk, int head_dim,
                    float p_drop, unsigned long long seed, const unsigned long long* seed_dev, unsigned site, int b_offset,
                    void* drop_mask_bits, hriemo_stream_t stream);
int hriemo_attn_bwd(const void* Q, long ldq, const void* K, long ldk, const void* V, long ldv, const void* O, long ldo,
                    const void* dO, long lddo, void* dQ, long lddq, void* dK, long lddk, void* dV, long lddv,
                    const unsigned char* key_padding_mask, const float* lse, float* delta, int B, int H, int Lq,
                    int Lk, int head_dim, float p_drop, unsigned long long seed, const unsigned long long* seed_dev,
                    unsigned site, int b_offset, float* dq_colsum_partials, float* dkv_colsum_partials,
                    const void* drop_mask_bits, hriemo_stream_t stream);
long hriemo_attn_mask_bytes(int B, int H, int Lq, int Lk);
int hriemo_attn_bwd_single_pass(int B, int H, int Lk, int head_dim);
int hriemo_attn_bwd_single_pass_q(int B, int H, int Lq, int Lk, int head_dim);
int hriemo_attn_bwd_kv_colsum_rows(int B, int H, int Lq, int Lk, int head_dim);
int hriemo_attn_plan(int B, int H, int Lq, int Lk, int head_dim, int cus, int* fwd_rows, int* bwd_form, int* dq_rows, int* dkv_rows,
                     int* dq_colsum_rows, int* kv_colsum_rows);
int hriemo_attn_fwd_q(const void* Q, long ldq, const void* K, long ldk, const void* V, long ldv, void* O, long ldo,
                      const unsigned char* key_padding_mask, float* lse, int B, int H, int Lq, int Lk, int head_dim, float p_drop,
                      unsigned long long seed, const unsigned long long* seed_dev, unsigned site, int b_offset, void* drop_mask_bits,
                      void* Oq, long ldoq, void* So, long ldso, hriemo_stream_t stream);
int hriemo_attn_fwd_varlen(const void* Q, long ldq, const void* K, long ldk, const void* V, long ldv, void* O, long ldo,
                           const int* cu_seqlens_q, const int* cu_seqlens_k, float* lse, int B, int H, int max_len_q,
                           int max_len_k, int head_dim, float p_drop, unsigned long long seed, const unsigned long long* seed_dev,
                           unsigned site, int b_offset, void* drop_mask_bits, hriemo_stream_t stream);
int hriemo_attn_fwd_q_varlen(const void* Q, long ldq, const void* K, long ldk, const void* V, long ldv, void* O, long ldo,
                             const int* cu_seqlens_q, const int* cu_seqlens_k, float* lse, int B, int H, int max_len_q,
                             int max_len_k, int head_dim, float p_drop, unsigned long long seed, const unsigned long long* seed_dev,
                             unsigned site, int b_offset, void* drop_mask_bits, void* Oq, long ldoq, void* So, long ldso,
                             long n_rows, hriemo_stream_t stream);
int hriemo_attn_bwd_varlen(const void* Q, long ldq, const void* K, long ldk, const void* V, long ldv, const void* O, long ldo,
                           const void* dO, long lddo, void* dQ, long lddq, void* dK, long lddk, void* dV, long lddv,
                           const int* cu_seqlens_q, const int* cu_seqlens_k, const float* lse, float* delta, int B, int H,
                           int max_len_q, int max_len_k, int head_dim, float p_drop, unsigned long long seed,
                           const unsigned long long* seed_dev, unsigned site, int b_offset, float* dq_colsum_partials,
                           float* dkv_colsum_partials, const void* drop_mask_bits, hriemo_stream_t stream);
int hriemo_attn_bwd_colsum_rows(int B, int H, int L, int head_dim);
int hriemo_attn_bwd_dq_colsum_rows(int B, int H, int Lq, int Lk, int head_dim);
int hriemo_attn_probs(const void* Q, long ldq, const void* K, long ldk, const unsigned char* key_padding_mask,
                      const float* lse, float* probs, int B, int H, int Lq, int Lk, int head_dim, float p_drop,
                      unsigned long long seed, const unsigned long long* seed_dev, unsigned site, int b_offset,
                      hriemo_stream_t stream);
int hriemo_attn_probs_varlen(const void* Q, long ldq, const void* K, long ldk, const int* cu_seqlens_q, const int* cu_seqlens_k,
                             const float* lse, float* probs, int B, int H, int max_len_q, int max_len_k, int out_lq, int out_lk,
                             int head_dim, float p_drop, unsigned long long seed, const unsigned long long* seed_dev, unsigned site,
                             int b_offset, hriemo_stream_t stream);
int hriemo_attn_probs_mfma(const void* Q, long ldq, const void* K, long ldk, const unsigned char* key_padding_mask,
                           const float* lse, float* probs, int B, int H, int Lq, int Lk, int head_dim, float p_drop,
                           unsigned long long seed, const unsigned long long* seed_dev, unsigned site, int b_offset,
                           hriemo_stream_t stream);

int hriemo_add_ln_fwd(const void* G, const void* X, const float* X32, const float* gamma, const float* beta, void* Y,
                      float* Y32, float* mean, float* rstd, int M, int d, float eps, float p_drop, unsigned long long seed,
                      const unsigned long long* seed_dev, unsigned site, long row_offset, hriemo_stream_t stream);
int hriemo_add_ln_fwd_mx8(const void* G, const void* X, const float* X32, const float* gamma, const float* beta, void* Y,
                          float* Y32, float* mean, float* rstd, int M, int d, float eps, float p_drop, unsigned long long seed,
                          const unsigned long long* seed_dev, unsigned site, long row_offset, void* Yq, void* SY, long ldsy,
                          hriemo_stream_t stream);
int hriemo_add_ln_fwd_rows(const void* G, const void* X, const float* X32, const float* gamma, const float* beta, void* Y,
                           float* Y32, float* mean, float* rstd, int M, int d, float eps, float p_drop, unsigned long long seed,
                           const unsigned long long* seed_dev, unsigned site, long row_offset, void* Yq, void* SY, long ldsy,
                           const long long* row_index, hriemo_stream_t stream);
// ... 2 lines not shown
                           int M, int d, float p_drop, unsigned long long seed, const unsigned long long* seed_dev,
                           unsigned site, long row_offset, float* workspace, const long long* row_index, hriemo_stream_t stream);
int hriemo_pack_rows(const void* X16, const float* X32, const int* cu_seqlens, int B, int L, int d, int n_rows, void* P16, float* P32,
                     long long* row_index, hriemo_stream_t stream);
int hriemo_unpack_rows(const void* P16, const float* P32, const int* cu_seqlens, int B, int L, int d, void* Y16, float* Y32,
                       hriemo_stream_t stream);
long hriemo_add_ln_bwd_workspace_bytes(int M, int d);
int hriemo_add_ln_bwd(const void* dY, const void* G, const void* X, const float* X32, const float* gamma, const float* mean,
                      const float* rstd, void* dX, void* dG, float* dgamma, float* dbeta, float* dbias, int accumulate,
                      int M, int d, float p_drop, unsigned long long seed, const unsigned long long* seed_dev,
                      unsigned site, long row_offset, float* workspace, hriemo_stream_t stream);

long hriemo_colsum_workspace_bytes(int M, int N);
int hriemo_colsum_bf16(const void* X, long ldx, int M, int N, float* out, int accumulate, float* workspace,
                       hriemo_stream_t stream);
int hriemo_cast_f32_to_bf16(const float* src, void* dst, long n, hriemo_stream_t stream);
int hriemo_cast_bf16_to_f32(const void* src, float* dst, long n, hriemo_stream_t stream);
int hriemo_cast_f32_to_bf16_batch(const void* jobs_host, int njobs, hriemo_stream_t stream);
int hriemo_cast_copy_batch(const void* jobs_host, int njobs, hriemo_stream_t stream);
int hriemo_dropout_bf16(const void* X, void* Y, long M, int N, float p_drop, unsigned long long seed,
                        const unsigned long long* seed_dev, unsigned site, long row_offset, hriemo_stream_t stream);
int hriemo_expand_rows(const float* q, void* out, float* out32, int B, long n, hriemo_stream_t stream);
int hriemo_seed_bump(unsigned long long* seed_dev, hriemo_stream_t stream);
int hriemo_rowdot_fwd(const void* Z, const float* Z32, const float* w, const float* b, float* out, int M, int d,
                      hriemo_stream_t stream);
int hriemo_rowdot_bwd(const float* dl, const void* Z, const float* Z32, const float* w, void* dZ, float* dw, float* db, int accumulate,
                      int M, int d, hriemo_stream_t stream);

int hriemo_pool_chunks(int L);
int hriemo_ln_pool_fwd(const void* X, const float* X32, const unsigned char* mask, const float* gamma, const float* beta, void* Yn,
                       float* mean, float* rstd, float* partials, int B, int L, int Lkeep, int d, float eps,
                       hriemo_stream_t stream);
int hriemo_gate_input(const float* partials_a, const float* partials_t, const unsigned char* mask_a,
                      const unsigned char* mask_t, int B, int La, int Lt, int d, void* gate_in, float* a_pool,
                      float* t_pool, float* cnt, hriemo_stream_t stream);
int hriemo_sigmoid_beta(const float* pre, float* w, float* beta, int B, int d, hriemo_stream_t stream);
int hriemo_fuse_fwd(const float* w, const void* A, const void* T, void* H, int B, int L, int d, hriemo_stream_t stream);
int hriemo_fuse_bwd_dw(const void* dH, const void* A, const void* T, float* partials, int B, int L, int d,
                       hriemo_stream_t stream);
int hriemo_gate_dpre(const float* partials, int L, const float* dbeta, const float* w, void* dpre, int B, int d,
                     hriemo_stream_t stream);
int hriemo_gate_input_bwd(const void* dgin, const float* a_pool, const float* t_pool, const float* cnt, float* da,
                          float* dt, int B, int d, hriemo_stream_t stream);
int hriemo_masked_mean_fwd(const void* X, const unsigned char* mask, float* pooled, float* cnt, int B, int L, int d,
                           hriemo_stream_t stream);
int hriemo_rowsum_f32(const float* x, float* out, int B, long n, hriemo_stream_t stream);
int hriemo_gate_input_pooled(const float* a_pool, const float* t_pool, void* gate_in, int B, int d, hriemo_stream_t stream);
int hriemo_fusion_loss(const float* logits, const float* targets, const float* pos_weight, const float* beta, int B, int Ne,
                       int reg_mode, float reg_coef, float scale, float* loss, float* dlogits, float* dbeta, hriemo_stream_t stream);
int hriemo_fusion_loss_ce(const float* logits, const long long* labels, const float* beta, int B, int C, int reg_mode,
                          float reg_coef, float scale, float* loss, float* dlogits, float* dbeta, hriemo_stream_t stream);
int hriemo_scalar_gate_dx(const void* dH, int Lf, const float* beta, int is_a, const float* dpool, const float* cnt,
                          const unsigned char* mask, void* dX, int B, int L, int d, hriemo_stream_t stream);
int hriemo_sumsq_f32(const float* x, long n, float* partial, int nblocks, hriemo_stream_t stream);
int hriemo_adamw_flat(float* p, const float* g, float* m, float* v, long n, float lr, float beta1, float beta2, float eps,
                      float weight_decay, int step, float max_norm, const float* norm2, hriemo_stream_t stream);
int hriemo_optim_finalize(const float* partial, int nblocks, const float* hyper, const float* grad_scale, const float* found_inf,
                          float* state, hriemo_stream_t stream);
int hriemo_adamw_flat_dev(float* p, const float* g, float* m, float* v, long n, const float* hyper, const float* state,
                          hriemo_stream_t stream);
int hriemo_add_ln_bwd_partial_rows(int M, int d);
int hriemo_rowops_force_variant(int variant);
int hriemo_colsum_partial_rows(int M, int N);
int hriemo_colreduce_batch(const void* jobs_host, int njobs, void* jobs_dev, int nblocks, hriemo_stream_t stream);
int hriemo_debug_hog(int blocks, int micros, float* sink, hriemo_stream_t stream);
int hriemo_ln_pool_pair_supported(int d);
int hriemo_ln_pool_fwd_pair(const void* Xa, const float* Xa32, const unsigned char* mask_a, const float* gamma_a, const float* beta_a,
                            void* Yna, float* mean_a, float* rstd_a, float* partials_a, int La,
                            const void* Xt, const float* Xt32, const unsigned char* mask_t, const float* gamma_t, const float* beta_t,
                            void* Ynt, float* mean_t, float* rstd_t, float* partials_t, int Lt,
                            int B, int Lkeep, int d, float eps, hriemo_stream_t stream);
int hriemo_ln_pool_bwd_pair(const void* dH, int Lf, const float* w,
                            const float* dpool_a, const unsigned char* mask_a, const void* Xa, const float* Xa32, const float* gamma_a,
                            const float* mean_a, const float* rstd_a, void* dXa, float* dgamma_a, float* dbeta_a, int La, float* workspace_a,
                            const float* dpool_t, const unsigned char* mask_t, const void* Xt, const float* Xt32, const float* gamma_t,
                            const float* mean_t, const float* rstd_t, void* dXt, float* dgamma_t, float* dbeta_t, int Lt, float* workspace_t,
                            int accumulate, int B, int d, hriemo_stream_t stream);
int hriemo_ln_pool_bwd_chunks(int L);
long hriemo_ln_pool_bwd_workspace_bytes(int B, int L, int d);
int hriemo_ln_pool_bwd(const void* dH, int Lf, const float* w, int is_a, const float* dpool, const unsigned char* mask,
                       const void* X, const float* X32, const float* gamma, const float* mean, const float* rstd, void* dX,
                       float* dgamma, float* dbeta, int accumulate, int B, int L, int d, float* workspace, hriemo_stream_t stream);

int hriemo_ln_pool_fwd_packed(const void* X, const float* X32, const int* cu_seqlens, int nseq, int n_rows, const float* gamma,
                              const float* beta, void* Yn, float* mean, float* rstd, float* partials, int L,
                              const int* cu_fused, int n_fused, int B, int d, float eps, hriemo_stream_t stream);
int hriemo_ln_pool_fwd_packed_pair(const void* Xa, const float* Xa32, const int* cu_a, int nseq_a, int n_rows_a, const float* gamma_a,
                                   const float* beta_a, void* Yna, float* mean_a, float* rstd_a, float* partials_a, int La,
                                   const void* Xt, const float* Xt32, const int* cu_t, int nseq_t, int n_rows_t, const float* gamma_t,
                                   const float* beta_t, void* Ynt, float* mean_t, float* rstd_t, float* partials_t, int Lt,
                                   const int* cu_fused, int n_fused, int B, int d, float eps, hriemo_stream_t stream);
int hriemo_fuse_fwd_packed(const float* w, const void* A, const void* T, void* H, const int* cu_fused, int n_fused, int B, int L, int d,
                           hriemo_stream_t stream);
int hriemo_fuse_fwd_packed_q(const float* w, const void* A, const void* T, void* H, const int* cu_fused, int n_fused, int B, int L, int d,
                             void* Hq, void* Hs, long lds, hriemo_stream_t stream);
int hriemo_fuse_bwd_dw_packed(const void* dH, const void* A, const void* T, float* partials, const int* cu_fused, int n_fused, int B,
                              int L, int d, hriemo_stream_t stream);
int hriemo_ln_pool_bwd_packed(const void* dH, const int* cu_fused, int n_fused, const float* w, int is_a, const float* dpool,
                              const void* X, const float* X32, const int* cu_seqlens, int nseq, int n_rows, const float* gamma,
                              const float* mean, const float* rstd, void* dX, float* dgamma, float* dbeta, int accumulate, int B, int L,
                              int d, float* workspace, hriemo_stream_t stream);
int hriemo_ln_pool_bwd_packed_pair(const void* dH, const int* cu_fused, int n_fused, const float* w,
                                   const float* dpool_a, const void* Xa, const float* Xa32, const int* cu_a, int nseq_a, int n_rows_a,
                                   const float* gamma_a, const float* mean_a, const float* rstd_a, void* dXa, float* dgamma_a,
                                   float* dbeta_a, int La, float* workspace_a,
                                   const float* dpool_t, const void* Xt, const float* Xt32, const int* cu_t, int nseq_t, int n_rows_t,
                                   const float* gamma_t, const float* mean_t, const float* rstd_t, void* dXt, float* dgamma_t,
                                   float* dbeta_t, int Lt, float* workspace_t, int accumulate, int B, int d, hriemo_stream_t stream);

int hriemo_split_bf16x3(const float* X, long ldx, int M, int K, void* Y, int layout, int relu, hriemo_stream_t stream);
int hriemo_attn_fwd_f32(const float* Q, long ldq, const float* K, long ldk, const float* V, long ldv, float* O, long ldo,
                        const unsigned char* key_padding_mask, float* lse, int B, int H, int Lq, int Lk, int head_dim,
                        float p_drop, unsigned long long seed, const unsigned long long* seed_dev, unsigned site, int b_offset,
                        hriemo_stream_t stream);
int hriemo_attn_probs_f32(const float* Q, long ldq, const float* K, long ldk, const unsigned char* key_padding_mask,
                          const float* lse, float* probs, int B, int H, int Lq, int Lk, int head_dim, float p_drop,
                          unsigned long long seed, const unsigned long long* seed_dev, unsigned site, int b_offset,
                          hriemo_stream_t stream);
int hriemo_add_ln_f32(const float* G, const float* X, const float* gamma, const float* beta, float* Y32, void* Y16, int M, int d,
                      float eps, float p_drop, unsigned long long seed, const unsigned long long* seed_dev, unsigned site,
                      long row_offset, hriemo_stream_t stream);
int hriemo_dropout_f32(const float* X, float* Y, long M, int N, int relu, const float* gate, float p_drop, unsigned long long seed,
                       const unsigned long long* seed_dev, unsigned site, long row_offset, hriemo_stream_t stream);
int hriemo_masked_mean_f32(const float* X, const unsigned char* mask, float* pooled, int B, int L, int d, hriemo_stream_t stream);
int hriemo_gate_input_f32(const float* a_pool, const float* t_pool, float* gate_in, int B, int d, hriemo_stream_t stream);
int hriemo_sigmoid_beta_f32(const float* pre, float* w, float* beta, int B, int d, hriemo_stream_t stream);
int hriemo_fuse_f32(const float* w, const float* A, int La, const float* T, int Lt, float* H32, void* H16, int B, int L, int d,
                    hriemo_stream_t stream);

int hriemo_split3_f32(const float* X, long ldx, int M, int K, void* Y, int form, int relu, const float* mask, long ldmask,
                      hriemo_stream_t stream);
long hriemo_colsum_f32_workspace_bytes(int M, int N);
int hriemo_colsum_f32(const float* X, long ldx, int M, int N, const float* mask, long ldmask, float* out, int accumulate,
                      float* workspace, hriemo_stream_t stream);
long hriemo_add_ln_bwd_f32_workspace_bytes(int M, int d);
int hriemo_add_ln_bwd_f32(const float* dY, const float* G, const float* X, const float* gamma, float* dS, float* dG, float* dgamma,
                          float* dbeta, float* dbias, int accumulate, int M, int d, float eps, float p_drop, unsigned long long seed,
                          const unsigned long long* seed_dev, unsigned site, long row_offset, float* workspace, hriemo_stream_t stream);
int hriemo_attn_bwd_f32(const float* Q, long ldq, const float* K, long ldk, const float* V, long ldv, const float* O, long ldo,
                        const float* dO, long lddo, const unsigned char* key_padding_mask, const float* lse, float* dQ, long lddq,
                        float* dK, long lddk, float* dV, long lddv, float* delta, int B, int H, int Lq, int Lk, int head_dim,
                        float p_drop, unsigned long long seed, const unsigned long long* seed_dev, unsigned site, int b_offset,
                        hriemo_stream_t stream);
int hriemo_gate_dpre_f32(const float* dH, const float* A, int La, const float* T, int Lt, const float* w, const float* dbeta, float* dpre,
                         int B, int L, int d, hriemo_stream_t stream);
int hriemo_gate_input_bwd_f32(const float* dgin, const float* a_pool, const float* t_pool, float* da, float* dt, int B, int d,
                              hriemo_stream_t stream);
int hriemo_gate_dy_f32(const float* dH, const float* w, int is_a, const float* dpool, const unsigned char* mask, float* dY, int B, int L,
                       int Lx, int d, hriemo_stream_t stream);
int hriemo_rowdot_bwd_f32(const float* dl, const float* Z, const float* w, float* dZ, float* dw, float* db, int accumulate, int M, int d,
                          hriemo_stream_t stream);

int hriemo_attn_fwd_f32_varlen(const float* Q, long ldq, const float* K, long ldk, const float* V, long ldv, float* O, long ldo,
                               const int* cu_seqlens_q, const int* cu_seqlens_k, float* lse, int B, int H, int max_len_q, int max_len_k,
                               int head_dim, float p_drop, unsigned long long seed, const unsigned long long* seed_dev, unsigned site,
                               int b_offset, hriemo_stream_t stream);
int hriemo_attn_bwd_f32_varlen(const float* Q, long ldq, const float* K, long ldk, const float* V, long ldv, const float* O, long ldo,
                               const float* dO, long lddo, const int* cu_seqlens_q, const int* cu_seqlens_k, const float* lse, float* dQ,
                               long lddq, float* dK, long lddk, float* dV, long lddv, float* delta, int B, int H, int max_len_q,
                               int max_len_k, int head_dim, float p_drop, unsigned long long seed, const unsigned long long* seed_dev,
                               unsigned site, int b_offset, hriemo_stream_t stream);
int hriemo_attn_probs_f32_varlen(const float* Q, long ldq, const float* K, long ldk, const int* cu_seqlens_q, const int* cu_seqlens_k,
                                 const float* lse, float* probs, int B, int H, int max_len_q, int max_len_k, int out_lq, int out_lk,
                                 int head_dim, float p_drop, unsigned long long seed, const unsigned long long* seed_dev, unsigned site,
                                 int b_offset, hriemo_stream_t stream);
int hriemo_add_ln_f32_rows(const float* G, const float* X, const float* gamma, const float* beta, float* Y32, void* Y16, int M, int d,
// ... 33 lines not shown
```

Measured before the change: 8798 utterances/s.

## Fuse FFN dropout into GEMM epilogues and gate LayerNorm+pool into last add-LN

Adds a GEMM variant whose epilogue applies ReLU plus row dropout in the FFN forward and the dropout mask in the masked dX backward. This removes separate dropout kernels and their extra bf16 round trips. Separately, the last fusion layer's residual add+LayerNorm now also computes the beta-gate's LayerNorm and pooling partials in one kernel, which the gate stage picks up through a context registry instead of re-reading the activations. This adds cross-module coupling through the tensor-identity registry and new template instantiations that may raise register pressure.

```diff
diff --git a/hri-emo_amd/_lib.py b/hri-emo_amd/_lib.py
--- a/hri-emo_amd/_lib.py
+++ b/hri-emo_amd/_lib.py
@@ -15,6 +15,8 @@
     "hriemo_gemm_plan": ("iiiiiilppp", "i"),
     "hriemo_gemm_bf16_group_tn": ("piip", "i"),
     "hriemo_gemm_bf16_split": ("iiiiiplplplpliiplp", "i"),
+    "hriemo_gemm_rowdrop_supported": ("iiii", "i"),
+    "hriemo_gemm_bf16_rowdrop": ("iiiiplplplpiplplfQpIlp", "i"),
     "hriemo_gemm_bf16_colsum": ("iiiiiplplplplpp", "i"),
     "hriemo_mx8_scale_ld": ("i", "l"),
     "hriemo_quant_mx8": ("pliiiplplp", "i"),
@@ -113,6 +115,8 @@
     "hriemo_ln_pool_pair_supported": ("i", "i"),
     "hriemo_ln_pool_fwd_pair": ("pppppppppi" * 2 + "iiifp", "i"),
     "hriemo_ln_pool_bwd_pair": ("pip" + "ppppppppppip" * 2 + "iiip", "i"),
+    "hriemo_add_ln_pool_supported": ("i", "i"),
+    "hriemo_add_ln_pool_fwd": ("ppppppppp" + "ffQpIl" + "ppppppp" + "iiiifp", "i"),
     "hriemo_ln_pool_bwd_workspace_bytes": ("iii", "l"),
     "hriemo_ln_pool_bwd": ("pipipppppppppp" + "iiiipp", "i"),
     "hriemo_ln_pool_fwd_packed": ("pppiippppppipiiifp", "i"),
diff --git a/hri-emo_amd/_ops.py b/hri-emo_amd/_ops.py
--- a/hri-emo_amd/_ops.py
+++ b/hri-emo_amd/_ops.py
@@ -75,10 +75,11 @@
 
 
 class StepContext:
-    __slots__ = ("capturing", "capture_origin", "seq_override", "join_scope", "half_reports")
+    __slots__ = ("capturing", "capture_origin", "seq_override", "join_scope", "half_reports", "gate_norm")
 
     def __init__(self):
         self.capturing, self.capture_origin, self.seq_override, self.join_scope, self.half_reports = False, None, None, 0, {}
+        self.gate_norm = {}
 
 
 CTX = StepContext()
@@ -461,6 +462,37 @@
     return dx
 
 
+FFN_ROWDROP = _os.environ.get("HRIEMO_FFN_ROWDROP", "1") != "0"
+
+
+def set_ffn_rowdrop(on):
+    global FFN_ROWDROP
+    FFN_ROWDROP = bool(on)
+
+
+def ffn_rowdrop(tb, M, N, K):
+    return FFN_ROWDROP and gemm_mode() == "bf16" and bool(_lib.lib().hriemo_gemm_rowdrop_supported(tb, M, N, K))
+
+
+def linear_relu_drop_fwd(x, w16, bias, p, seed, site, row_off):
+    M, K = x.shape
+    N = w16.shape[0]
+    h = torch.empty((M, N), dtype=BF16, device=x.device)
+    hd = torch.empty((M, N), dtype=BF16, device=x.device)
+    _lib.call("hriemo_gemm_bf16_rowdrop", 0, M, N, K, _p(x), x.stride(0), _p(w16), w16.stride(0), _p(h), N, _p(bias), 1, None, 0,
+              _p(hd), N, float(p), seed, _p(seed_word(x.device)), site, row_off, _stream())
+    return h, hd
+
+
+def linear_dx_masked_drop(dy, w16, aux, p, seed, site, row_off):
+    M, N = dy.shape
+    K = w16.shape[1]
+    dx = torch.empty((M, K), dtype=BF16, device=dy.device)
+    _lib.call("hriemo_gemm_bf16_rowdrop", 1, M, K, N, _p(dy), dy.stride(0), _p(w16), w16.stride(0), _p(dx), K, None, 2, _p(aux),
+              aux.stride(0), None, 0, float(p), seed, _p(seed_word(dy.device)), site, row_off, _stream())
+    return dx
+
+
 FOLD_FFN_BIAS = True
 
 
@@ -875,6 +907,51 @@
     else:
         side = lambda x, x32, sx, *rest: (_p(x), _p(x32), _p(sx.kpm), *map(_p, rest), sx.L)
         _lib.call("hriemo_ln_pool_fwd_pair", *side(*a), *side(*t), a[2].B, sf.L, d, _EPS, _stream())
+
+
+GATE_FUSE_LN = _os.environ.get("HRIEMO_GATE_FUSE_LN", "1") != "0"
+
+
+def set_gate_fuse_ln(on):
+    global GATE_FUSE_LN
+    GATE_FUSE_LN = bool(on)
+
+
+def gate_fuse_ln():
+    return GATE_FUSE_LN
+
+
+class GateNorm:
+    __slots__ = ("gamma", "beta", "kpm", "Lkeep", "out")
+
+    def __init__(self, gamma, beta, kpm, Lkeep):
+        self.gamma, self.beta, self.kpm, self.Lkeep, self.out = gamma, beta, kpm, Lkeep, None
+
+    def take(self, x, gamma, beta, kpm, Yn_shape):
+        o, self.out = self.out, None
+        if o is None or gamma is not self.gamma or beta is not self.beta or _p(kpm) != _p(self.kpm):
+            return None
+        if o[0].data_ptr() != x.data_ptr() or o[0].numel() != x.numel() or tuple(o[1].shape) != tuple(Yn_shape):
+            return None
+        return o
+
+
+def add_ln_pool_fwd(g, x, gamma, beta, p, seed, site, row_off, x32, want32, gn, B, L):
+    M, d = g.shape
+    dev = g.device
+    f32 = dict(dtype=torch.float32, device=dev)
+    y = torch.empty((M, d), dtype=BF16, device=dev)
+    y32 = torch.empty((M, d), **f32) if want32 else None
+    mean, rstd = torch.empty(M, **f32), torch.empty(M, **f32)
+    Yn = torch.empty((B, gn.Lkeep, d), dtype=BF16, device=dev)
+    mean_g, rstd_g = torch.empty(M, **f32), torch.empty(M, **f32)
+    part = torch.empty((B, _lib.lib().hriemo_pool_chunks(L), d), **f32)
+    if DROP_LOG is not None and p > 0:
+        DROP_LOG.append(("rows", seed, site, M, d, float(p), row_off))
+    _lib.call("hriemo_add_ln_pool_fwd", _p(g), _p(x), _p(x32), _p(gamma), _p(beta), _p(y), _p(y32), _p(mean), _p(rstd), _EPS, float(p),
+              seed, _p(seed_word(dev)), site, row_off, _p(gn.kpm), _p(gn.gamma), _p(gn.beta), _p(Yn), _p(mean_g), _p(rstd_g), _p(part),
+              B, L, gn.Lkeep, d, _EPS, _stream())
+    return (y, y32, mean, rstd), (Yn, mean_g, rstd_g, part)
 
 
 def fuse_fwd(w, An, Tn, H, sf, d):
@@ -1760,15 +1837,29 @@
         x32 = _c32(x32)
         x32v = x32.view(M, d) if x32 is not None else None
         w1_16, w2_16 = sh.get(w1), sh.get(w2)
-        h = proj_fwd(Operand(x2, mx_of(x)), sh, w1, w1_16, b1, relu=True, want_q=p_mid == 0)
-        hd_ = h
-        if p_mid > 0:
+        F = w1.shape[0]
+        if p_mid > 0 and DROP_LOG is not None:
+            DROP_LOG.append(("rows", seed, site + 2, M, F, float(p_mid), b_off * L))
+        if p_mid > 0 and ffn_rowdrop(0, M, F, d):
+            h, hd_ = linear_relu_drop_fwd(x2, w1_16, b1, p_mid, seed, site + 2, b_off * L)
+        else:
+            h = proj_fwd(Operand(x2, mx_of(x)), sh, w1, w1_16, b1, relu=True, want_q=p_mid == 0)
+            hd_ = h
+        if p_mid > 0 and hd_ is h:
             hd_ = torch.empty_like(h)
-            if DROP_LOG is not None:
-                DROP_LOG.append(("rows", seed, site + 2, M, h.shape[1], float(p_mid), b_off * L))
             _lib.call("hriemo_dropout_bf16", _p(h), _p(hd_), M, h.shape[1], float(p_mid), seed, _p(seed_word(h.device)),
                       site + 2, b_off * L, _stream())
-        g, y, y32, mean, rstd, mx = _proj_ln(hd_, sh, w2, w2_16, b2, x2, x32v, gamma, beta, p, seed, site + 1, b_off * seq.L, seq.idx)
+        gn = CTX.gate_norm.get(id(gamma)) if CTX.gate_norm else None
+        if gn is not None and (seq.packed or gn.Lkeep > L or fuse_ln(M, d) or want_mx_copy(M, d)
+                               or not _lib.lib().hriemo_add_ln_pool_supported(d)):
+            gn = None
+        if gn is not None:
+            g = proj_fwd(Operand(hd_, mx_of(hd_)), sh, w2, w2_16, b2)
+            (y, y32, mean, rstd), dep = add_ln_pool_fwd(g, x2, gamma, beta, p, seed, site + 1, b_off * seq.L, x32v, TWIN, gn, B, L)
+            gn.out = (y,) + dep + (torch.cuda.current_stream(x2.device),)
+            mx = None
+        else:
+            g, y, y32, mean, rstd, mx = _proj_ln(hd_, sh, w2, w2_16, b2, x2, x32v, gamma, beta, p, seed, site + 1, b_off * seq.L, seq.idx)
         ctx.save_for_backward(x2, x32v, h, hd_, g, mean, rstd, w1_16, w2_16, gamma)
         ctx.cfg = (B, L, d, p, p_mid, seed, site, b_off)
         ctx.seq = seq
@@ -1791,11 +1882,14 @@
         linear_dw(dg, hd_, dw2, acc)
         db1 = sink.buf(p_b1)
         fold = p_mid == 0 and fold_ffn_bias()
+        drop_in_gemm = p_mid > 0 and ffn_rowdrop(1, M, F, d)
         if fold:
             da = linear_dx_masked_colsum(dg, w2_16, h, db1, acc)
+        elif drop_in_gemm:
+            da = linear_dx_masked_drop(dg, w2_16, h, p_mid, seed, site + 2, b_off * L)
         else:
             da = linear_dx(dg, w2_16, epi=2, aux=h)
-        if p_mid > 0:
+        if p_mid > 0 and not drop_in_gemm:
             _lib.call("hriemo_dropout_bf16", _p(da), _p(da), M, F, float(p_mid), seed, _p(seed_word(dev)), site + 2, b_off * L,
                       _stream())
         dw1 = sink.buf(p_w1)
@@ -1831,17 +1925,32 @@
         f32 = dict(dtype=torch.float32, device=dev)
         L_ = _lib.lib()
         nca, nct = L_.hriemo_pool_chunks(La), L_.hriemo_pool_chunks(Lt)
-        An = torch.empty(sf.shape(d), dtype=BF16, device=dev)
-        Tn = torch.empty(sf.shape(d), dtype=BF16, device=dev)
-        mean_a, rstd_a = torch.empty(Ra, **f32), torch.empty(Ra, **f32)
-        mean_t, rstd_t = torch.empty(Rt, **f32), torch.empty(Rt, **f32)
-        pa, pt = torch.empty((B, nca, d), **f32), torch.empty((B, nct, d), **f32)
         st_ = _stream()
+        main = torch.cuda.current_stream(dev)
+        dep_a = dep_t = None
+        gna, gnt = (CTX.gate_norm.get(id(ga)), CTX.gate_norm.get(id(gt))) if CTX.gate_norm else (None, None)
+        if gna is not None and gnt is not None and not sf.packed:
+            dep_a, dep_t = gna.take(xa, ga, ba, sa.kpm, sf.shape(d)), gnt.take(xt, gt, bt, st.kpm, sf.shape(d))
+        fused = dep_a is not None and dep_t is not None
+        if fused:
+            (_, An, mean_a, rstd_a, pa, sda), (_, Tn, mean_t, rstd_t, pt, sdt) = dep_a, dep_t
+            if not CTX.capturing:
+                for ts_, sd_ in ((dep_a[1:5], sda), (dep_t[1:5], sdt)):
+                    if sd_ != main:
+                        for t_ in ts_:
+                            share(t_, main)
+        else:
+            An = torch.empty(sf.shape(d), dtype=BF16, device=dev)
+            Tn = torch.empty(sf.shape(d), dtype=BF16, device=dev)
+            mean_a, rstd_a = torch.empty(Ra, **f32), torch.empty(Ra, **f32)
+            mean_t, rstd_t = torch.empty(Rt, **f32), torch.empty(Rt, **f32)
+            pa, pt = torch.empty((B, nca, d), **f32), torch.empty((B, nct, d), **f32)
         side_a = (xa, h_a32, sa, ga, ba, An, mean_a, rstd_a, pa)
         side_t = (xt, h_t32, st, gt, bt, Tn, mean_t, rstd_t, pt)
-        main = torch.cuda.current_stream(dev)
         side = side_stream(dev) if GATE_TWO_STREAMS else None
-        if GATE_PAIR and L_.hriemo_ln_pool_pair_supported(d):
+        if fused:
+            pass
+        elif GATE_PAIR and L_.hriemo_ln_pool_pair_supported(d):
             ln_pool_fwd_pair(side_a, side_t, sf, d)
         elif side is not None and side != main:
             fork(side, main)
diff --git a/hri-emo_amd/csrc/gemm.hip b/hri-emo_amd/csrc/gemm.hip
--- a/hri-emo_amd/csrc/gemm.hip
+++ b/hri-emo_amd/csrc/gemm.hip
@@ -2,8 +2,8 @@
 #include <string.h>
 #include <stdlib.h>
 
-template <int TA, int TB, int OUTF32, int BM, int BN, int WM, int WN, int NS, int BK>
-__device__ __forceinline__ void gemm_body(const GemmArgs& p) {
+template <int TA, int TB, int OUTF32, int BM, int BN, int WM, int WN, int NS, int BK, int RD = 0>
+__device__ __forceinline__ void gemm_body(const GemmArgs& p, const GemmDrop& rd = GemmDrop{}) {
   constexpr int NWAVE = WM * WN;
   constexpr bool K32 = (BK == 32), STAG = K32 && (WM * WN == 8);
   constexpr int A_BYTES = BM * BK * 2, B_BYTES = BN * BK * 2, STAGE = A_BYTES + B_BYTES;
@@ -324,7 +324,11 @@
     if (skip_epilogue) {
     } else
 #endif
-    if (OUTF32) {
+    if constexpr (RD == 1) {
+      store_tile<0, 1, MT, NTL, 1>(acc, p, T, scratch, wm, wn, lane, rd);
+    } else if constexpr (RD == 2) {
+      store_tile<0, 2, MT, NTL, 2>(acc, p, T, scratch, wm, wn, lane, rd);
+    } else if (OUTF32) {
       store_tile<1, 0, MT, NTL>(acc, p, T, scratch, wm, wn, lane);
     } else {
       switch (p.epi) {
@@ -337,7 +341,7 @@
     if (!has_next) break;
     if (!OUTF32) {
       const int rows_valid = p.M - (T.m0 + wm * MT * 16), cols_valid = p.N - (T.n0 + wn * 64);
-      relax_first = (p.flags & 1) && rows_valid >= MT * 16 && cols_valid >= 64 && p.cs == nullptr;
+      relax_first = RD == 0 && (p.flags & 1) && rows_valid >= MT * 16 && cols_valid >= 64 && p.cs == nullptr;
     }
     T = decode(nwg);
     wg = nwg;
@@ -355,6 +359,10 @@
 template <int TA, int TB, int OUTF32, int BM, int BN, int WM, int WN, int NS, int BK>
 __global__ __launch_bounds__(WM * WN * 64, (WM * WN == 4 ? 2 : 1)) void gemm_kernel(const GemmArgs p) {
   gemm_body<TA, TB, OUTF32, BM, BN, WM, WN, NS, BK>(p);
+}
+template <int TB, int RD, int BM, int BN, int WM, int WN, int NS, int BK>
+__global__ __launch_bounds__(WM * WN * 64, (WM * WN == 4 ? 2 : 1)) void gemm_rowdrop_kernel(const GemmArgs p, const GemmDrop rd) {
+  gemm_body<0, TB, 0, BM, BN, WM, WN, NS, BK, RD>(p, rd);
 }
 
 template <int TA, int TB, int OUTF32>
@@ -791,6 +799,81 @@
   return 0;
 }
 
+template <int TB, int RD, int BM, int BN, int WM, int WN, int NS>
+static void launch_rowdrop(const GemmArgs& a, const GemmDrop& rd, int ring, hipStream_t st) {
+  const int lds = ring + WM * WN * 2048;
+  static bool attr_set = false;
+  if (!attr_set) {
+    hipFuncSetAttribute((const void*)gemm_rowdrop_kernel<TB, RD, BM, BN, WM, WN, NS, 64>, hipFuncAttributeMaxDynamicSharedMemorySize, lds);
+    attr_set = true;
+  }
+  const long units = (long)a.tiles_m * a.tiles_n;
+  const long slots = (long)hriemo_num_cus() * (lds <= 80 * 1024 ? 2 : 1);
+  GemmArgs q = a;
+  q.sched = units > slots ? hriemo_gemm_sched_slot(st) : nullptr;
+  hipLaunchKernelGGL((gemm_rowdrop_kernel<TB, RD, BM, BN, WM, WN, NS, 64>), dim3((int)(units < slots ? units : slots)), dim3(WM * WN * 64), lds, st, q, rd);
+}
+static bool rowdrop_cfg(int cfg) { return cfg == 0 || cfg == 3 || cfg == 7 || cfg == 8; }
+extern "C" int hriemo_gemm_rowdrop_supported(int tb, int M, int N, int K) {
+  if (M <= 0 || N <= 0 || K <= 0 || (tb != 0 && tb != 1)) return 0;
+  return rowdrop_cfg(plan_gemm(0, tb, M, N, K, 0, 0).cfg) ? 1 : 0;
+}
+extern "C" int hriemo_gemm_bf16_rowdrop(int tb, int M, int N, int K, const void* A, long lda, const void* B, long ldb, void* C, long ldc,
+                                        const float* bias, int epilogue, const void* aux, long ldaux, void* D, long ldd, float p_drop,
+                                        unsigned long long seed, const unsigned long long* seed_dev, unsigned site, long row_offset,
+                                        hipStream_t st) {
+  HRIEMO_CHECK(M > 0 && N > 0 && K > 0, "gemm_rowdrop: empty problem M=%d N=%d K=%d", M, N, K);
+  HRIEMO_CHECK((epilogue == 1 && tb == 0) || (epilogue == 2 && tb == 1),
+               "gemm_rowdrop: built for the FFN's forward (tb=0, epilogue 1) and its masked dX (tb=1, epilogue 2); got tb=%d epilogue=%d", tb, epilogue);
+  HRIEMO_CHECK(N % 8 == 0 && K % 8 == 0, "gemm_rowdrop: N=%d and K=%d must be multiples of 8", N, K);
+  HRIEMO_CHECK(A != nullptr && B != nullptr && C != nullptr, "gemm_rowdrop: A, B and C are required");
+  HRIEMO_CHECK(lda % 8 == 0 && ldb % 8 == 0 && ldc % 8 == 0, "gemm_rowdrop: leading dims must keep 16-byte alignment");
+  HRIEMO_CHECK(((uintptr_t)A % 16) == 0 && ((uintptr_t)B % 16) == 0 && ((uintptr_t)C % 16) == 0, "gemm_rowdrop: unaligned operand");
+  HRIEMO_CHECK(lda < (1L << 21) && ldb < (1L << 21), "gemm_rowdrop: leading dimension too large for 32-bit tile offsets");
+  HRIEMO_CHECK(lda >= K && ldb >= (tb ? N : K) && ldc >= N, "gemm_rowdrop: a leading dimension is shorter than its row");
+  HRIEMO_CHECK(p_drop >= 0.f && p_drop < 1.f, "gemm_rowdrop: p_drop=%g outside [0, 1)", (double)p_drop);
+  if (epilogue == 1) {
+    HRIEMO_CHECK(D != nullptr && ldd % 8 == 0 && ldd >= N && ((uintptr_t)D % 16) == 0, "gemm_rowdrop: epilogue 1 needs a 16-byte aligned D with ldd >= N");
+  } else {
+    HRIEMO_CHECK(D == nullptr, "gemm_rowdrop: epilogue 2 drops C in place, D must be NULL");
+    HRIEMO_CHECK(aux != nullptr && ldaux % 8 == 0 && ldaux >= N && ((uintptr_t)aux % 16) == 0, "gemm_rowdrop: epilogue 2 needs a 16-byte aligned aux");
+    HRIEMO_CHECK(bias == nullptr, "gemm_rowdrop: the masked dX has no bias");
+  }
+  const GemmPlan pl = plan_gemm(0, tb, M, N, K, 0, 0);
+  const int cfg = pl.cfg;
+  HRIEMO_CHECK(rowdrop_cfg(cfg) && pl.splitk == 1, "gemm_rowdrop: %dx%dx%d is not a decoder-sized problem (hriemo_gemm_rowdrop_supported); use "
+               "hriemo_gemm_bf16 + hriemo_dropout_bf16", M, N, K);
+  GemmArgs a = {};
+  a.M = M; a.N = N; a.K = K;
+  a.A = (const bf16_t*)A; a.lda = lda; a.B = (const bf16_t*)B; a.ldb = ldb;
+  a.C = C; a.ldc = ldc; a.bias = bias; a.aux = (const bf16_t*)aux; a.ldaux = ldaux; a.epi = epilogue;
+  a.tiles_m = (M + kCfg[cfg].bm - 1) / kCfg[cfg].bm; a.tiles_n = (N + kCfg[cfg].bn - 1) / kCfg[cfg].bn;
+  a.flags = g_gemm_flags;
+  a.splitk = 1; a.k_per_split = pl.k_per_split;
+  const DropCfg dc = make_drop(p_drop, seed, site);
+  const GemmDrop rd{(bf16_t*)D, ldd, seed, seed_dev, site, dc.thr16, dc.inv_keep, row_offset};
+  const int ring = kCfg[cfg].lds;
+  const int cls = tb ? HP_GEMM_NN : HP_GEMM_NT;
+  hriemo_prof_begin(cls, st);
+  if (tb == 0) {
+    switch (cfg) {
+      case 0: launch_rowdrop<0, 1, 128, 128, 2, 2, 2>(a, rd, ring, st); break;
+      case 7: launch_rowdrop<0, 1, 32, 128, 2, 2, 7>(a, rd, ring, st); break;
+      case 8: launch_rowdrop<0, 1, 32, 64, 2, 1, 6>(a, rd, ring, st); break;
+      default: launch_rowdrop<0, 1, 64, 128, 2, 2, 4>(a, rd, ring, st); break;
+    }
+  } else {
+    switch (cfg) {
+      case 0: launch_rowdrop<1, 2, 128, 128, 2, 2, 2>(a, rd, ring, st); break;
+      case 7: launch_rowdrop<1, 2, 32, 128, 2, 2, 7>(a, rd, ring, st); break;
+      default: launch_rowdrop<1, 2, 64, 128, 2, 2, 4>(a, rd, ring, st); break;
+    }
+  }
+  HRIEMO_LAUNCH_CHECK("gemm_rowdrop_kernel");
+  hriemo_prof_end(cls, st, 2.0 * M * N * K);
+  return 0;
+}
+
 extern "C" int hriemo_gemm_bf16(int ta, int tb, int M, int N, int K, const void* A, long lda, const void* B, long ldb,
                                 void* C, long ldc, int c_is_f32, const float* bias, int epilogue, const void* aux,
                                 long ldaux, int accumulate, float* workspace, long workspace_bytes, hipStream_t st) {
diff --git a/hri-emo_amd/csrc/gemm_common.h b/hri-emo_amd/csrc/gemm_common.h
--- a/hri-emo_amd/csrc/gemm_common.h
+++ b/hri-emo_amd/csrc/gemm_common.h
@@ -23,6 +23,13 @@
   uint8_t* SC; long ldsc;
 };
 
+struct GemmDrop {
+  bf16_t* D; long ldd;
+  uint64_t seed; const unsigned long long* seed_dev;
+  uint32_t site, thr16; float inv_keep;
+  long row_offset;
+};
+
 unsigned* hriemo_gemm_sched_slot(hipStream_t st);
 int hriemo_num_cus();
 int hriemo_gemm_debug_flags_get();
@@ -146,9 +153,10 @@
 typedef __attribute__((ext_vector_type(4))) short s16x4v;
 typedef __attribute__((ext_vector_type(8))) short s16x8v;
 
-template <int OUTF32, int EPI, int MT, int NTL>
+template <int OUTF32, int EPI, int MT, int NTL, int RD = 0>
 __device__ __forceinline__ void store_tile(f32x4 (&acc)[MT][NTL], const GemmArgs& p, const TileInfo& T, char* scratch,
-                                           int wm, int wn, int lane_in) {
+                                           int wm, int wn, int lane_in, const GemmDrop& rd = GemmDrop{}) {
+  static_assert(RD == 0 || (!OUTF32 && (EPI == 1 || EPI == 2)), "row dropout rides on the ReLU / ReLU-mask epilogues");
   static_assert(NTL == 4, "wave tiles are 64 columns wide");
   int lane = lane_in;
   asm volatile("" : "+v"(lane));
@@ -214,6 +222,16 @@
     const int wsw = i & 7, gh = g >> 1;
     const char* rd0 = scratch + rr * 128 + ((cc ^ rr) << 4);
     if (EPI >= 2) load_chunk(0, 0);
+    uint32_t dkey = 0;
+    char* dbase = nullptr;
+    unsigned line_d = 0;
+    if (RD != 0) {
+      dkey = rd.thr16 != 0 ? site_key(eff_seed(rd.seed, rd.seed_dev), rd.site, 0u) : 0u;
+      if (RD == 1) {
+        dbase = (char*)(rd.D + (long)mb * rd.ldd + nb);
+        line_d = (unsigned)((rr * rd.ldd + cc * 8) * 2);
+      }
+    }
     float cs8[EPI == 2 ? 8 : 1];
 #pragma unroll
     for (int e = 0; e < (EPI == 2 ? 8 : 1); ++e) cs8[e] = 0.f;
@@ -257,6 +275,23 @@
             }
           }
           const bool ok = mi * 16 + k * 8 + rr < rows_valid && cc * 8 < cols_valid;
+          if (RD != 0) {
+            const uint32_t hb = drop_base(dkey, (uint32_t)(rd.row_offset + mb + mi * 16 + k * 8 + rr), (uint32_t)((nb + cc * 8) >> 1));
+            float f8[8];
+            bf8_to_f32(__builtin_bit_cast(bf16x8, v), f8);
+#pragma unroll
+            for (int pr = 0; pr < 4; ++pr) {
+              const uint32_t x = mix24(hb + (uint32_t)pr * DROP_CB);
+              f8[2 * pr] = (rd.thr16 == 0 || keep_lo(x, rd.thr16)) ? f8[2 * pr] * rd.inv_keep : 0.f;
+              f8[2 * pr + 1] = (rd.thr16 == 0 || keep_hi(x, rd.thr16)) ? f8[2 * pr + 1] * rd.inv_keep : 0.f;
+            }
+            const u32x4 dv = __builtin_bit_cast(u32x4, f32_to_bf8(f8));
+            if (RD == 1) {
+              if (full || ok) *(u32x4*)(dbase + (long)((mi * 16 + k * 8) * rd.ldd * 2) + line_d) = dv;
+            } else {
+              v = dv;
+            }
+          }
           if (full || ok) *(u32x4*)(cbase + (long)((mi * 16 + k * 8) * p.ldc * 2) + line_c) = v;
           if (EPI <= 1 && p.CQ != nullptr) {
             float f8[8];
diff --git a/hri-emo_amd/csrc/rowops.hip b/hri-emo_amd/csrc/rowops.hip
--- a/hri-emo_amd/csrc/rowops.hip
+++ b/hri-emo_amd/csrc/rowops.hip
@@ -1,6 +1,7 @@
 #include "common.h"
 #include <string.h>
 #include <stdlib.h>
+#include <type_traits>
 
 #define EPS_DEFAULT 1e-5f
 
@@ -738,6 +739,282 @@
   ln_pool_fwd_body<NCH, PF, true>(PAIR_PICK(X), PAIR_PICK(X32), nullptr, PAIR_PICK(gamma), PAIR_PICK(beta), PAIR_PICK(Yn), PAIR_PICK(mean),
                                   PAIR_PICK(rstd), PAIR_PICK(partials), PAIR_PICK(L), 0, d, eps,
                                   (int)blockIdx.x - (second ? p.s[0].nc : 0), PAIR_PICK(nc), pk);
+}
+
+struct AddLnPoolArgs {
+  const bf16_t* G; const bf16_t* X; const float* X32; const float* gamma; const float* beta; bf16_t* Y; float* Y32; float* mean; float* rstd;
+  const uint8_t* mask; const float* gamma2; const float* beta2; bf16_t* Yn; float* mean2; float* rstd2; float* partials; int L, Lkeep;
+};
+template <int NCH>
+__global__ __launch_bounds__(256) void add_ln_pool_fwd_kernel(const AddLnPoolArgs a, int d, float eps, float eps2, RowDrop dr, long row_offset) {
+#pragma clang fp contract(off)
+  extern __shared__ __attribute__((aligned(16))) char smem_raw[];
+  float* red = (float*)smem_raw;
+  float* cst = red + d;
+  const uint32_t key32 = row_key(dr);
+  const int lane = threadIdx.x & 63, wave = threadIdx.x >> 6;
+  const int b = blockIdx.y, chunk = blockIdx.x, nchunks = gridDim.x, nchunk = d >> 3;
+  const int L = a.L, Lkeep = a.Lkeep;
+  const long xbase = (long)b * L, ybase = (long)b * Lkeep;
+  const float invd = 1.f / (float)d;
+  const bf16_t* __restrict__ G = a.G;
+  const bf16_t* __restrict__ X = a.X;
+  const float* __restrict__ X32 = a.X32;
+  bf16_t* __restrict__ Y = a.Y;
+  float* __restrict__ Y32 = a.Y32;
+  bf16_t* __restrict__ Yn = a.Yn;
+  for (int t = threadIdx.x; t < d; t += 256) { cst[t] = a.gamma2[t]; cst[d + t] = a.beta2[t]; }
+  __syncthreads();
+  float acc[NCH][8], gm8[NCH][8], bt8[NCH][8];
+#pragma unroll
+  for (int c = 0; c < NCH; ++c)
+#pragma unroll
+    for (int j = 0; j < 8; ++j) acc[c][j] = 0.f;
+  load_cols<NCH>(a.gamma, nchunk, lane, gm8);
+  load_cols<NCH>(a.beta, nchunk, lane, bt8);
+  const int lend = min(L, chunk * 32 + 32);
+  bf16x8 ng[NCH];
+  float nx[NCH][8];
+  auto load_row = [&](int l) {
+#pragma unroll
+    for (int c = 0; c < NCH; ++c) {
+      const int ch = lane + 64 * c;
+      if (ch < nchunk) {
+        ng[c] = *(const bf16x8*)(G + (xbase + l) * d + ch * 8);
+        load_resid(X, X32, (xbase + l) * d + ch * 8, nx[c]);
+      }
+    }
+  };
+#pragma unroll
+  for (int c = 0; c < NCH; ++c) {
+    ng[c] = bf16x8{};
+#pragma unroll
+    for (int j = 0; j < 8; ++j) nx[c][j] = 0.f;
+  }
+  if (chunk * 32 + wave < lend) load_row(chunk * 32 + wave);
+  for (int l = chunk * 32 + wave; l < lend; l += 4) {
+    const long row = xbase + l;
+    float s[NCH][8];
+    float sum = 0.f;
+#pragma unroll
+    for (int c = 0; c < NCH; ++c) {
+      const int ch = lane + 64 * c;
+      if (ch < nchunk) {
+        float gf[8];
+        bf8_to_f32(ng[c], gf);
+        bool kp8[8];
+        row_keep8(key32, dr.thr16, (uint32_t)(row_offset + (long)row), ch, kp8);
+#pragma unroll
+        for (int j = 0; j < 8; ++j) {
+          const float gv = kp8[j] ? gf[j] * dr.inv_keep : 0.f;
+          s[c][j] = nx[c][j] + gv;
+          sum += s[c][j];
+        }
+      } else {
+#pragma unroll
+        for (int j = 0; j < 8; ++j) s[c][j] = 0.f;
+      }
+    }
+    if (l + 4 < lend) load_row(l + 4);
+    const float mu = wave_sum(sum) * invd;
+    float sq = 0.f;
+#pragma unroll
+    for (int c = 0; c < NCH; ++c)
+      if (lane + 64 * c < nchunk) {
+#pragma unroll
+        for (int j = 0; j < 8; ++j) { const float t = s[c][j] - mu; sq += t * t; }
+      }
+    const float rstd = rsqrtf(__builtin_fmaf(wave_sum(sq), invd, eps));
+    float sum2 = 0.f;
+#pragma unroll
+    for (int c = 0; c < NCH; ++c) {
+      const int ch = lane + 64 * c;
+      if (ch < nchunk) {
+        float o[8];
+#pragma unroll
+        for (int j = 0; j < 8; ++j) o[j] = __builtin_fmaf((s[c][j] - mu) * rstd, gm8[c][j], bt8[c][j]);
+        const bf16x8 ob = f32_to_bf8(o);
+        *(bf16x8*)(Y + row * d + ch * 8) = ob;
+        if (Y32 != nullptr) {
+          *(f32x4*)(Y32 + row * d + ch * 8) = (f32x4){o[0], o[1], o[2], o[3]};
+          *(f32x4*)(Y32 + row * d + ch * 8 + 4) = (f32x4){o[4], o[5], o[6], o[7]};
+        } else {
+          bf8_to_f32(ob, o);
+        }
+#pragma unroll
+        for (int j = 0; j < 8; ++j) { s[c][j] = o[j]; sum2 += s[c][j]; }
+      }
+    }
+    if (lane == 0) { a.mean[row] = mu; a.rstd[row] = rstd; }
+    const float mu2 = wave_sum(sum2) * invd;
+    float sq2 = 0.f;
+#pragma unroll
+    for (int c = 0; c < NCH; ++c)
+      if (lane + 64 * c < nchunk) {
+#pragma unroll
+        for (int j = 0; j < 8; ++j) { const float t = s[c][j] - mu2; sq2 += t * t; }
+      }
+    const float rstd2 = rsqrtf(__builtin_fmaf(wave_sum(sq2), invd, eps2));
+    const bool valid = a.mask == nullptr || a.mask[row] == 0;
+#pragma unroll
+    for (int c = 0; c < NCH; ++c) {
+      const int ch = lane + 64 * c;
+      if (ch < nchunk) {
+        float o[8];
+#pragma unroll
+        for (int j = 0; j < 8; ++j) {
+          o[j] = __builtin_fmaf((s[c][j] - mu2) * rstd2, cst[ch * 8 + j], cst[d + ch * 8 + j]);
+          if (valid) acc[c][j] += o[j];
+        }
+        if (l < Lkeep) *(bf16x8*)(Yn + (ybase + l) * d + ch * 8) = f32_to_bf8(o);
+      }
+    }
+    if (lane == 0) { a.mean2[row] = mu2; a.rstd2[row] = rstd2; }
+  }
+  block_colsum<NCH>(red, acc, nchunk, lane, wave, 4);
+  float* out = a.partials + ((long)b * nchunks + chunk) * d;
+  for (int t = threadIdx.x; t < d; t += 256) out[t] = red[t];
+}
+
+template <int NCH>
+struct RowOps { bf16x8 g[NCH]; f32x4 x[NCH][2]; };
+template <int NCH>
+__global__ __launch_bounds__(256, 4) void add_ln_pool_fwd_twin_kernel(const AddLnPoolArgs a, int d, float eps, float eps2, RowDrop dr, long row_offset) {
+#pragma clang fp contract(off)
+  extern __shared__ __attribute__((aligned(16))) char smem_raw[];
+  float* red = (float*)smem_raw;
+  float* cst = red + d;
+  const uint32_t key32 = row_key(dr);
+  const int lane = threadIdx.x & 63;
+  const int wave = __builtin_amdgcn_readfirstlane(threadIdx.x >> 6);
+  const int b = blockIdx.y, chunk = blockIdx.x, nchunks = gridDim.x, nchunk = d >> 3;
+  const int L = a.L, Lkeep = a.Lkeep;
+  const long xbase = (long)b * L, ybase = (long)b * Lkeep;
+  const float invd = 1.f / (float)d;
+  const bf16_t* __restrict__ G = a.G;
+  const float* __restrict__ X32 = a.X32;
+  bf16_t* __restrict__ Y = a.Y;
+  float* __restrict__ Y32 = a.Y32;
+  bf16_t* __restrict__ Yn = a.Yn;
+  float* __restrict__ mean_o = a.mean;
+  float* __restrict__ rstd_o = a.rstd;
+  float* __restrict__ mean2_o = a.mean2;
+  float* __restrict__ rstd2_o = a.rstd2;
+  for (int t = threadIdx.x; t < d; t += 256) { cst[t] = a.gamma[t]; cst[d + t] = a.beta[t]; cst[2 * d + t] = a.gamma2[t]; cst[3 * d + t] = a.beta2[t]; }
+  __syncthreads();
+  float acc[NCH][8];
+  bool on[NCH];
+  int co[NCH];
+#pragma unroll
+  for (int c = 0; c < NCH; ++c) {
+    on[c] = lane + 64 * c < nchunk;
+    co[c] = on[c] ? (lane + 64 * c) * 8 : 0;
+#pragma unroll
+    for (int j = 0; j < 8; ++j) acc[c][j] = 0.f;
+  }
+  const int l0 = chunk * 32 + wave, lend = min(L, chunk * 32 + 32);
+  if (l0 < lend) {
+    const int llast = l0 + ((lend - 1 - l0) >> 2) * 4;
+    auto load_row = [&](int l, RowOps<NCH>& r) {
+      const long o = (xbase + l) * d;
+#pragma unroll
+      for (int c = 0; c < NCH; ++c) {
+        r.g[c] = *(const bf16x8*)(G + o + co[c]);
+        r.x[c][0] = *(const f32x4*)(X32 + o + co[c]);
+        r.x[c][1] = *(const f32x4*)(X32 + o + co[c] + 4);
+      }
+    };
+    RowOps<NCH> cur, nx1;
+    load_row(l0, cur);
+    int mflag = 0;
+    if (a.mask != nullptr) mflag = a.mask[xbase + min(l0 + 4 * (lane & 7), llast)];
+    auto step = [&](int l, auto keep_tag) {
+      constexpr bool KEEP = decltype(keep_tag)::value;
+      const long row = xbase + l;
+      load_row(min(l + 4, llast), nx1);
+      const uint32_t hrow = (uint32_t)(row_offset + row);
+      float s[NCH][8];
+      float sum = 0.f;
+#pragma unroll
+      for (int c = 0; c < NCH; ++c) {
+        float gf[8];
+        bf8_to_f32(cur.g[c], gf);
+        const uint32_t hb = drop_base(key32, hrow, (uint32_t)(co[c] >> 1));
+        bool kp8[8];
+#pragma unroll
+        for (int pr = 0; pr < 4; ++pr) {
+          const uint32_t x = mix24(hb + (uint32_t)pr * DROP_CB);
+          kp8[2 * pr] = dr.thr16 == 0 || keep_lo(x, dr.thr16);
+          kp8[2 * pr + 1] = dr.thr16 == 0 || keep_hi(x, dr.thr16);
+        }
+#pragma unroll
+        for (int j = 0; j < 8; ++j) {
+          const float gv = kp8[j] ? gf[j] * dr.inv_keep : 0.f;
+          s[c][j] = cur.x[c][j >> 2][j & 3] + gv;
+          if (on[c]) sum += s[c][j];
+        }
+      }
+      const float mu = wave_sum(sum) * invd;
+      float sq = 0.f;
+#pragma unroll
+      for (int c = 0; c < NCH; ++c)
+        if (on[c]) {
+#pragma unroll
+          for (int j = 0; j < 8; ++j) { const float t = s[c][j] - mu; sq += t * t; }
+        }
+      const float rstd = rsqrtf(__builtin_fmaf(wave_sum(sq), invd, eps));
+      float sum2 = 0.f;
+      int lo[NCH];
+#pragma unroll
+      for (int c = 0; c < NCH; ++c) { lo[c] = co[c]; asm volatile("" : "+v"(lo[c])); }
+#pragma unroll
+      for (int c = 0; c < NCH; ++c) {
+        float o[8];
+#pragma unroll
+        for (int j = 0; j < 8; ++j) o[j] = __builtin_fmaf((s[c][j] - mu) * rstd, cst[lo[c] + j], cst[d + lo[c] + j]);
+        *(bf16x8*)(Y + row * d + co[c]) = f32_to_bf8(o);
+        *(f32x4*)(Y32 + row * d + co[c]) = (f32x4){o[0], o[1], o[2], o[3]};
+        *(f32x4*)(Y32 + row * d + co[c] + 4) = (f32x4){o[4], o[5], o[6], o[7]};
+#pragma unroll
+        for (int j = 0; j < 8; ++j) {
+          s[c][j] = o[j];
+          if (on[c]) sum2 += s[c][j];
+        }
+      }
+      mean_o[row] = mu;
+      rstd_o[row] = rstd;
+      const float mu2 = wave_sum(sum2) * invd;
+      float sq2 = 0.f;
+#pragma unroll
+      for (int c = 0; c < NCH; ++c)
+        if (on[c]) {
+#pragma unroll
+          for (int j = 0; j < 8; ++j) { const float t = s[c][j] - mu2; sq2 += t * t; }
+        }
+      const float rstd2 = rsqrtf(__builtin_fmaf(wave_sum(sq2), invd, eps2));
+      const bool valid = __builtin_amdgcn_readlane(mflag, (l - l0) >> 2) == 0;
+#pragma unroll
+      for (int c = 0; c < NCH; ++c) {
+        float o[8];
+#pragma unroll
+        for (int j = 0; j < 8; ++j) {
+          o[j] = __builtin_fmaf((s[c][j] - mu2) * rstd2, cst[2 * d + lo[c] + j], cst[3 * d + lo[c] + j]);
+          if (valid && on[c]) acc[c][j] += o[j];
+        }
+        if (KEEP) *(bf16x8*)(Yn + (ybase + l) * d + co[c]) = f32_to_bf8(o);
+      }
+      mean2_o[row] = mu2;
+      rstd2_o[row] = rstd2;
+      cur = nx1;
+    };
+    int l = l0;
+    const int lk = min(lend, Lkeep);
+    for (; l < lk; l += 4) step(l, std::true_type{});
+    for (; l < lend; l += 4) step(l, std::false_type{});
+  }
+  block_colsum<NCH>(red, acc, nchunk, lane, wave, 4);
+  float* out = a.partials + ((long)b * nchunks + chunk) * d;
+  for (int t = threadIdx.x; t < d; t += 256) out[t] = red[t];
 }
 
 __global__ __launch_bounds__(256) void gate_input_kernel(const float* __restrict__ pa, int nca, const float* __restrict__ pt, int nct,
@@ -1657,6 +1934,38 @@
   else hipLaunchKernelGGL((ln_pool_fwd_pair_kernel<2, true>), dim3(nc, B), dim3(256), d * 4, st, p, d, eps);
   HRIEMO_LAUNCH_CHECK("ln_pool_fwd_pair_kernel");
   hriemo_prof_end(HP_ROWOPS, st, ((double)B * (La + Lt) + 2.0 * B * Lkeep) * d * 2);
+  return 0;
+}
+
+extern "C" int hriemo_add_ln_pool_supported(int d) { return hriemo_ln_pool_pair_supported(d) && !use_quad(d) ? 1 : 0; }
+extern "C" int hriemo_add_ln_pool_fwd(const void* G, const void* X, const float* X32, const float* gamma, const float* beta, void* Y,
+                                      float* Y32, float* mean, float* rstd, float eps, float p_drop, unsigned long long seed,
+                                      const unsigned long long* seed_dev, unsigned site, long row_offset, const unsigned char* mask,
+                                      const float* gamma_g, const float* beta_g, void* Yn, float* mean_g, float* rstd_g, float* partials,
+                                      int B, int L, int Lkeep, int d, float eps_g, hipStream_t st) {
+  HRIEMO_CHECK(B > 0 && L > 0 && (long)B * L <= 0x7fffffffL, "add_ln_pool_fwd: B=%d, L=%d is not a row count", B, L);
+  if (check_rows(B * L, d)) return 1;
+  HRIEMO_CHECK(Lkeep >= 0 && Lkeep <= L, "add_ln_pool_fwd: Lkeep=%d out of range (L=%d)", Lkeep, L);
+  HRIEMO_CHECK(hriemo_add_ln_pool_supported(d), "add_ln_pool_fwd: d=%d (built for d <= 1024 and the chunk-mapped add_ln kernels; use "
+               "hriemo_add_ln_fwd + hriemo_ln_pool_fwd)", d);
+  HRIEMO_CHECK(G != nullptr && gamma != nullptr && beta != nullptr && Y != nullptr && mean != nullptr && rstd != nullptr,
+               "add_ln_pool_fwd: G, gamma, beta, Y, mean and rstd are required");
+  HRIEMO_CHECK(gamma_g != nullptr && beta_g != nullptr && Yn != nullptr && mean_g != nullptr && rstd_g != nullptr && partials != nullptr,
+               "add_ln_pool_fwd: the gate's gamma, beta, Yn, mean, rstd and partials are required");
+  const RowDrop dr = row_drop(p_drop, seed, seed_dev, site);
+  const AddLnPoolArgs a{(const bf16_t*)G, (const bf16_t*)X, X32, gamma, beta, (bf16_t*)Y, Y32, mean, rstd,
+                        mask, gamma_g, beta_g, (bf16_t*)Yn, mean_g, rstd_g, partials, L, Lkeep};
+  const int nc = (L + 31) / 32;
+  hriemo_prof_begin(HP_ROWOPS, st);
+  if (X32 != nullptr && Y32 != nullptr) {
+    if (d <= 512) hipLaunchKernelGGL((add_ln_pool_fwd_twin_kernel<1>), dim3(nc, B), dim3(256), 5 * d * 4, st, a, d, eps, eps_g, dr, row_offset);
+    else hipLaunchKernelGGL((add_ln_pool_fwd_twin_kernel<2>), dim3(nc, B), dim3(256), 5 * d * 4, st, a, d, eps, eps_g, dr, row_offset);
+  } else {
+    if (d <= 512) hipLaunchKernelGGL((add_ln_pool_fwd_kernel<1>), dim3(nc, B), dim3(256), 3 * d * 4, st, a, d, eps, eps_g, dr, row_offset);
+    else hipLaunchKernelGGL((add_ln_pool_fwd_kernel<2>), dim3(nc, B), dim3(256), 3 * d * 4, st, a, d, eps, eps_g, dr, row_offset);
+  }
+  HRIEMO_LAUNCH_CHECK("add_ln_pool_fwd_kernel");
+  hriemo_prof_end(HP_ROWOPS, st, (((X32 ? 3.0 : (X ? 2.0 : 1.0)) + 1.0 + (Y32 ? 2.0 : 0.0)) * B * L + (double)B * Lkeep) * d * 2);
   return 0;
 }
 
diff --git a/hri-emo_amd/models/fusion_with_emotion_decoder.py b/hri-emo_amd/models/fusion_with_emotion_decoder.py
--- a/hri-emo_amd/models/fusion_with_emotion_decoder.py
+++ b/hri-emo_amd/models/fusion_with_emotion_decoder.py
@@ -45,6 +45,18 @@
             ev.record(side)
         return ev
 
+    def _announce_gate_norms(self, h_a, h_t, mask_a, mask_t, need):
+        g = _ops.CTX.gate_norm
+        g.clear()
+        if not _ops.gate_fuse_ln() or need or _ops.precision() != "bf16" or len(self.cross_modal.layers) == 0:
+            return
+        if any(m is not None and m.dtype != torch.bool for m in (mask_a, mask_t)) or h_a.size(1) < h_t.size(1):
+            return
+        B, La, Lt = h_a.size(0), h_a.size(1), h_t.size(1)
+        last, bg = self.cross_modal.layers[-1], self.beta_gate
+        g[id(last.norm_a2.weight)] = g[id(bg.norm_a.weight)] = _ops.GateNorm(bg.norm_a.weight, bg.norm_a.bias, _ops.mask_u8(mask_a, B, La), Lt)
+        g[id(last.norm_t2.weight)] = g[id(bg.norm_t.weight)] = _ops.GateNorm(bg.norm_t.weight, bg.norm_t.bias, _ops.mask_u8(mask_t, B, Lt), Lt)
+
     def _ensure_3d(self, x):
         if x.dim() == 2:
             return x.unsqueeze(1)
@@ -82,13 +94,15 @@
         fused_early = None if may_pack else self._build_fused_mask(mask_a, mask_t, h_t.size(1))
         ready = self._prefetch_shadows(a.device)
         _ops.CTX.join_scope += 1
+        self._announce_gate_norms(h_a, h_t, mask_a, mask_t, need)
         try:
             a, a32, t, t32, encoder_attns, seqs = self.cross_modal._fwd_pair(a, a32, t, t32, mask_a, mask_t, need, tail=True)
+            if ready is not None:
+                torch.cuda.current_stream(a.device).wait_event(ready)
+            h_fusion, beta = self.beta_gate._fwd_pair(a, a32, t, t32, mask_a, mask_t, seqs)
         finally:
             _ops.CTX.join_scope -= 1
-        if ready is not None:
-            torch.cuda.current_stream(a.device).wait_event(ready)
-        h_fusion, beta = self.beta_gate._fwd_pair(a, a32, t, t32, mask_a, mask_t, seqs)
+            _ops.CTX.gate_norm.clear()
         sm = seqs[2]
         if not sm.packed:
             sm = sm.with_kpm(fused_early if (fused_early is not None and h_fusion.size(1) == h_t.size(1)) else
diff --git a/include/hriemo.h b/include/hriemo.h
--- a/include/hriemo.h
+++ b/include/hriemo.h
@@ -15,6 +15,11 @@
                      long ldaux, int accumulate, float* workspace, long workspace_bytes, hriemo_stream_t stream);
 
 int hriemo_gemm_bf16_group_tn(const void* jobs_host, int njobs, int accumulate, hriemo_stream_t stream);
+int hriemo_gemm_rowdrop_supported(int tb, int M, int N, int K);
+int hriemo_gemm_bf16_rowdrop(int tb, int M, int N, int K, const void* A, long lda, const void* B, long ldb, void* C, long ldc,
+                             const float* bias, int epilogue, const void* aux, long ldaux, void* D, long ldd, float p_drop,
+                             unsigned long long seed, const unsigned long long* seed_dev, unsigned site, long row_offset,
+                             hriemo_stream_t stream);
 int hriemo_gemm_bf16_split(int ta, int tb, int M, int N, int K, const void* A, long lda, const void* B, long ldb, void* C, long ldc,
                            void* C2, long ldc2, int split_m, int accumulate, float* workspace, long workspace_bytes,
                            hriemo_stream_t stream);
@@ -183,6 +188,13 @@
                        const void* X, const float* X32, const float* gamma, const float* mean, const float* rstd, void* dX,
                        float* dgamma, float* dbeta, int accumulate, int B, int L, int d, float* workspace, hriemo_stream_t stream);
 
+int hriemo_add_ln_pool_supported(int d);
+int hriemo_add_ln_pool_fwd(const void* G, const void* X, const float* X32, const float* gamma, const float* beta, void* Y,
+                           float* Y32, float* mean, float* rstd, float eps, float p_drop, unsigned long long seed,
+                           const unsigned long long* seed_dev, unsigned site, long row_offset, const unsigned char* mask,
+                           const float* gamma_g, const float* beta_g, void* Yn, float* mean_g, float* rstd_g, float* partials,
+                           int B, int L, int Lkeep, int d, float eps_g, hriemo_stream_t stream);
+
 int hriemo_ln_pool_fwd_packed(const void* X, const float* X32, const int* cu_seqlens, int nseq, int n_rows, const float* gamma,
                               const float* beta, void* Yn, float* mean, float* rstd, float* partials, int L,
                               const int* cu_fused, int n_fused, int B, int d, float eps, hriemo_stream_t stream);
```

Result: no change. 8823 utterances/s, median of 2 (+0.3%).
